# AnastasiaBelenkii/tendermint

Measured on AMD Instinct MI355X. Metric: ed25519 verifies/sec at 1/2/4/8 GPUs + p50 VerifyCommit latency, 150 vals, higher is better.
Workload: dtype int32

## Files before the change

__graft_entry__.py:

```python
import os
import subprocess
import sys

REPO = os.path.dirname(os.path.abspath(__file__))


def build() -> None:
    env = dict(os.environ, PYTORCH_ROCM_ARCH="gfx950")
    subprocess.run(["make", "-s", "-C", os.path.join(REPO, "tendermint_amd", "csrc")], check=True, env=env)
    subprocess.run(["bash", os.path.join(REPO, "tools", "build_checks.sh")], check=True, env=env)
    subprocess.run(["make", "-s", "-C", os.path.join(REPO, "oracle")], check=True)
    subprocess.run(["make", "-s", "-C", os.path.join(REPO, "tendermint_amd", "testing", "csrc")], check=True)
    subprocess.run(["make", "-s", "-C", os.path.join(REPO, "tests", "native")], check=True)
    subprocess.run(["make", "-s", "-C", os.path.join(REPO, "tests", "native", "secp")], check=True)
    subprocess.run(["make", "-s", "-C", os.path.join(REPO, "tests", "native", "secpcomb")], check=True)
    subprocess.run(["make", "-s", "-C", os.path.join(REPO, "tests", "native", "merkle")], check=True)
    subprocess.run(["make", "-s", "-C", os.path.join(REPO, "tests", "native", "pcache")], check=True)
    subprocess.run(["make", "-s", "-C", os.path.join(REPO, "tests", "native", "colorder")], check=True)
    subprocess.run(["make", "-s", "-C", os.path.join(REPO, "tests", "native", "blocks")], check=True)
    subprocess.run(["make", "-s", "-C", os.path.join(REPO, "tests", "native", "voteext")], check=True)
    subprocess.run(["make", "-s", "-C", os.path.join(REPO, "tests", "native", "proofops")], check=True)
    subprocess.run(["make", "-s", "-C", os.path.join(REPO, "tests", "native", "stage")], check=True)
    subprocess.run(["make", "-s", "-C", os.path.join(REPO, "tests", "native", "results")], check=True)
    sys.path.insert(0, REPO)
    import tendermint_amd
    from tendermint_amd import _native
    _native.lib()


def smoke() -> None:
    sys.path.insert(0, REPO)
    sys.path.insert(0, os.path.join(REPO, "oracle"))
    import numpy as np
    import torch
    from tendermint_amd import _native
    from tendermint_amd.testing.factory import make_c2_batch
    import oracle_c

    assert torch.cuda.is_available(), "smoke() needs a GPU"
    ctx = _native.Context(1)
    b = make_c2_batch(1000, seed=7)
    ok_g, vec_g = ctx.ed25519_verify_batch(b.pk, b.sig, b.msg, b.off)
    ok_o, vec_o = oracle_c.ed25519_verify_packed(b.pk, b.sig, b.msg, b.off, threads=4)
    assert ok_g == ok_o and np.array_equal(vec_g, vec_o), "GPU validity vector differs from the oracle"
    info = _native.build_info()
    print(f"smoke ok: {int(vec_g.sum())}/{b.n} valid, bit-exact vs oracle; {info['version']} "
          f"(src digest of this tree {'matches' if info['src_match'] else 'DIFFERS: ' + info['src_digest_tree']})")


if __name__ == "__main__":
    build()
    smoke()
```

include/tmverify.h:

```cpp
#ifndef TMVERIFY_H
#define TMVERIFY_H

#include <stddef.h>
#include <stdint.h>

#ifdef __cplusplus
extern "C" {
#endif

#define TMV_ALL_VALID 1
#define TMV_NOT_ALL 0
#define TMV_ERR_ARG (-1)
#define TMV_ERR_NO_DEVICE (-2)
#define TMV_ERR_NOMEM (-3)
#define TMV_ERR_LAUNCH (-4)
#define TMV_ERR_TIMEOUT (-5)
#define TMV_ERR_RANDOM (-6)

#define TMV_SR_ADDERR_PUBKEY (-1)
#define TMV_SR_ADDERR_SIG (-2)

#define TMV_KIND_ED25519 0
#define TMV_KIND_SR25519 1

// ... 9 lines not shown
int tmv_ed25519_verify_batch(tmv_ctx *ctx, const uint8_t *pk, const uint8_t *sig, const uint8_t *msg,
                             const uint32_t *msg_off, uint32_t n, uint8_t *valid_out);

int tmv_ed25519_verify(tmv_ctx *ctx, const uint8_t *pk, const uint8_t *msg, size_t msg_len,
                       const uint8_t *sig, size_t sig_len);

int tmv_secp256k1_verify_batch(tmv_ctx *ctx, const uint8_t *pk, const uint8_t *sig, const uint8_t *msg,
                               const uint32_t *msg_off, uint32_t n, uint8_t *valid_out);

int tmv_secp256k1_verify_batch_ex(tmv_ctx *ctx, uint32_t flags, const uint8_t *pk, const uint8_t *sig,
                                  const uint8_t *msg, const uint32_t *msg_off, uint32_t n, uint8_t *valid_out);
int tmv_secp256k1_key_cache_stats(tmv_ctx *ctx, uint64_t *hits, uint64_t *misses, uint32_t *used, uint32_t *capacity);

int tmv_secp256k1_verify(tmv_ctx *ctx, const uint8_t *pk, size_t pk_len, const uint8_t *msg, size_t msg_len,
                         const uint8_t *sig, size_t sig_len);

int tmv_sr25519_verify_batch(tmv_ctx *ctx, const uint8_t *pk, const uint8_t *sig, const uint8_t *msg,
                             const uint32_t *msg_off, uint32_t n, int8_t *status_out);

int tmv_verify_mixed_batch(tmv_ctx *ctx, const uint8_t *kind, const uint8_t *pk, const uint8_t *sig,
                           const uint8_t *msg, const uint32_t *msg_off, uint32_t n, int8_t *status_out);

#define TMV_FLAG_KEY_CACHE 1u
int tmv_verify_batch_ex(tmv_ctx *ctx, uint8_t key_kind, uint32_t flags, const uint8_t *pk, const uint8_t *sig,
                        const uint8_t *msg, const uint32_t *msg_off, uint32_t n, int8_t *status_out);
#define TMV_FLAG_BATCH_EQUATION 2u
#define TMV_FLAG_PER_ENTRY 4u
#define TMV_BATCHOPT_STATS 1u
#define TMV_BATCHOPT_SUBCHECK_ON 2u
#define TMV_BATCHOPT_SUBCHECK_OFF 4u
int tmv_set_batch_options(tmv_ctx *ctx, uint32_t group_log2, uint32_t window_bits, const uint8_t *seed32,
                          uint32_t opt_flags);
int tmv_batch_stats(tmv_ctx *ctx, uint64_t *groups, uint64_t *groups_failed);
int tmv_validator_set_hashes(tmv_ctx *ctx, const uint8_t *pk, const uint8_t *key_kind, const int64_t *power,
                             const uint32_t *set_off, uint32_t n_sets, uint8_t *hash_out);
int tmv_merkle_roots(tmv_ctx *ctx, const uint8_t *data, const uint32_t *leaf_off, uint32_t n_leaves,
                     const uint32_t *tree_off, uint32_t n_trees, uint8_t *hash_out);
int tmv_commit_hashes(tmv_ctx *ctx, const uint8_t *flag, const uint8_t *addr_len, const uint8_t *addr,
                      const int64_t *ts_seconds, const int32_t *ts_nanos, const uint8_t *sig_len, const uint8_t *sig,
                      const uint32_t *commit_off, uint32_t n_commits, uint8_t *hash_out);
#define TMV_RESULTS_FIRST_LEAF 1u
int tmv_tx_results_hashes(tmv_ctx *ctx, uint32_t flags, const uint32_t *code, const int64_t *gas_wanted,
                          const int64_t *gas_used, const uint8_t *data, const uint32_t *data_off,
                          const uint32_t *tree_off, uint32_t n_trees, const uint8_t *first, const uint32_t *first_off,
                          uint8_t *root_out);

#define TMV_MERKLE_PREHASH 1u
#define TMV_MERKLE_LEAF_HASH_GIVEN 2u
#define TMV_MERKLE_LONG_LEAVES 4u
#define TMV_MERKLE_SHORT_LEAVES 8u
#define TMV_MERKLE_LPW(l) ((uint32_t)(l) << 8)
int tmv_merkle_aunt_offsets(const uint32_t *tree_off, uint32_t n_trees, uint32_t *aunt_off_out);
int tmv_merkle_proofs(tmv_ctx *ctx, uint32_t flags, const uint8_t *data, const uint32_t *leaf_off, uint32_t n_leaves,
                      const uint32_t *tree_off, uint32_t n_trees, uint8_t *root_out, uint8_t *leaf_hash_out,
                      const uint32_t *aunt_off, uint8_t *aunts_out);
int tmv_merkle_verify_proofs(tmv_ctx *ctx, uint32_t flags, uint32_t n, const int64_t *total, const int64_t *index,
                             const uint8_t *leaf_hash, const uint8_t *aunts, const uint32_t *aunt_off,
                             const uint8_t *root, const uint8_t *data, const uint32_t *leaf_off, int8_t *status_out,
                             uint8_t *leaf_hash_calc, uint8_t *root_calc, uint8_t *root_nil);

int tmv_merkle_value_ops(tmv_ctx *ctx, uint32_t flags, uint32_t n_items, const uint8_t *value,
                         const uint32_t *value_off, const uint32_t *op_off, const uint8_t *key, const uint32_t *key_off,
                         const int64_t *total, const int64_t *index, const uint8_t *leaf_hash, const uint8_t *aunts,
                         const uint32_t *aunt_off, const uint8_t *root, uint8_t *value_digest, uint8_t *kv_hash_calc,
                         uint8_t *leaf_ok, uint8_t *root_calc, uint8_t *root_nil, int8_t *status_out,
                         int32_t *fail_op_out);

int tmv_subgroup_stats(tmv_ctx *ctx, uint64_t *subgroups, uint64_t *subgroups_failed);
int tmv_verify_mixed_batch_ex(tmv_ctx *ctx, uint32_t flags, const uint8_t *kind, const uint8_t *pk,
                              const uint8_t *sig, const uint8_t *msg, const uint32_t *msg_off, uint32_t n,
                              int8_t *status_out);

int tmv_kernel_timing(tmv_ctx *ctx, int enable);
int tmv_kernel_timing_read(tmv_ctx *ctx, const char *kernel, double *total_ms, uint64_t *launches);

int tmv_key_cache_stats(tmv_ctx *ctx, uint64_t *hits, uint64_t *misses, uint32_t *used, uint32_t *capacity);

int tmv_point_cache_stats(tmv_ctx *ctx, uint64_t *hits, uint64_t *misses, uint32_t *slots);

int tmv_bucket_entry_stats(tmv_ctx *ctx, uint64_t *entries);

int tmv_group_fail_stats(tmv_ctx *ctx, uint64_t *groups_failed, uint64_t *groups_located, uint64_t *fallback_entries);

typedef struct tmv_metrics {
  uint64_t calls;
  uint64_t signatures;
  uint64_t max_batch;
  uint64_t batch_eq_signatures;
  uint64_t host_signatures;
  double host_seconds;
  uint64_t h2d_bytes;
  uint64_t d2h_bytes;
  uint64_t groups;
  uint64_t groups_failed;
  uint64_t located_groups;
  uint64_t fallback_signatures;
  uint64_t key_cache_hits;
  uint64_t key_cache_misses;
} tmv_metrics;
int tmv_metrics_read(tmv_ctx *ctx, tmv_metrics *out);
int tmv_metrics_reset(tmv_ctx *ctx);

int tmv_ed25519_verify_batch_device(tmv_ctx *ctx, int device, const uint8_t *d_pk, const uint8_t *d_sig,
                                    const uint8_t *d_msg, const uint32_t *d_msg_off, uint32_t n,
                                    uint8_t *d_valid, void *stream);
int tmv_verify_mixed_batch_device(tmv_ctx *ctx, int device, const uint8_t *d_kind, const uint8_t *d_pk,
                                  const uint8_t *d_sig, const uint8_t *d_msg, const uint32_t *d_msg_off,
                                  uint32_t n, int8_t *d_status, void *stream);
#define TMV_KIND_MIXED 2
int tmv_verify_batch_device_ex(tmv_ctx *ctx, int device, uint8_t key_kind, uint32_t flags, const uint8_t *d_kind,
                               const uint8_t *d_pk, const uint8_t *d_sig, const uint8_t *d_msg,
                               const uint32_t *d_msg_off, uint32_t n, int8_t *d_status, void *stream);

#define TMV_MAX_BATCHES 256
typedef struct tmv_batch_ref {
  const uint8_t *pk;
  const uint8_t *sig;
  const uint8_t *msg;
  const uint32_t *msg_off;
  uint32_t n;
  uint32_t msg_bytes;
  int8_t *status;
} tmv_batch_ref;
int tmv_verify_batches_device(tmv_ctx *ctx, int device, uint8_t key_kind, uint32_t flags,
                              const tmv_batch_ref *batches, uint32_t n_batches, void *stream);

typedef struct tmv_vote_template {
  const uint8_t *head;
  uint32_t head_len;
  const uint8_t *block;
  uint32_t block_len;
  const uint8_t *chain;
  uint32_t chain_len;
} tmv_vote_template;

#define TMV_VOTE_WITH_BLOCK 0x80000000u

typedef struct tmv_vote {
  int64_t ts_seconds;
  int32_t ts_nanos;
  uint32_t tmpl;
} tmv_vote;

int tmv_verify_votes(tmv_ctx *ctx, uint8_t key_kind, uint32_t flags, const tmv_vote_template *tmpl,
                     uint32_t n_tmpl, const tmv_vote *votes, const uint8_t *pk, const uint8_t *sig, uint32_t n,
                     int8_t *status_out);

int64_t tmv_vote_sign_bytes_device(tmv_ctx *ctx, const tmv_vote_template *tmpl, uint32_t n_tmpl,
                                   const tmv_vote *votes, uint32_t n, uint8_t *msg_out, size_t msg_cap,
                                   uint32_t *msg_off_out);

typedef struct tmv_vote_ext_template { const uint8_t *tail; uint32_t tail_len; } tmv_vote_ext_template;

int tmv_verify_votes_and_extensions(tmv_ctx *ctx, uint8_t key_kind, uint32_t flags,
        const tmv_vote_template *tmpl, uint32_t n_tmpl, const tmv_vote *votes, uint32_t n_votes,
        const tmv_vote_ext_template *etmpl, uint32_t n_etmpl, const uint32_t *ext_tmpl,
        const uint8_t *ext_data, const uint32_t *ext_off, uint32_t n_exts,
        const uint8_t *pk, const uint8_t *sig, int8_t *status_out);
int64_t tmv_vote_extension_sign_bytes_device(tmv_ctx *ctx, const tmv_vote_ext_template *etmpl, uint32_t n_etmpl,
        const uint32_t *ext_tmpl, const uint8_t *ext_data, const uint32_t *ext_off, uint32_t n_exts,
        uint8_t *msg_out, size_t msg_cap, uint32_t *msg_off_out);

#ifdef __cplusplus
}
#endif
#endif
// ... 1 lines not shown
```

tendermint_amd/_native.py:

```python
from __future__ import annotations

import ctypes
import os
import subprocess
import threading

import numpy as np

_HERE = os.path.dirname(os.path.abspath(__file__))
LIB_PATH = os.environ.get("TMV_LIB_PATH") or os.path.join(_HERE, "_build", "libtmgpu.so")
HEADER_PATH = os.path.join(os.path.dirname(_HERE), "include", "tmverify.h")
HEADER_PATHS = [HEADER_PATH, os.path.join(os.path.dirname(_HERE), "include", "tmhost.h")]

TMV_ALL_VALID = 1
TMV_NOT_ALL = 0
TMV_ERR_ARG = -1
TMV_ERR_NO_DEVICE = -2
TMV_ERR_NOMEM = -3
TMV_ERR_LAUNCH = -4
TMV_SR_ADDERR_PUBKEY = -1
TMV_SR_ADDERR_SIG = -2
TMV_KIND_ED25519 = 0
TMV_KIND_SR25519 = 1
TMV_FLAG_KEY_CACHE = 1
TMV_FLAG_BATCH_EQUATION = 2
TMV_FLAG_PER_ENTRY = 4
TMV_BATCHOPT_STATS = 1
TMV_BATCHOPT_SUBCHECK_ON = 2
TMV_BATCHOPT_SUBCHECK_OFF = 4
TMV_MERKLE_PREHASH = 1
TMV_MERKLE_LEAF_HASH_GIVEN = 2
TMV_MERKLE_LONG_LEAVES = 4
TMV_MERKLE_SHORT_LEAVES = 8
TMV_RESULTS_FIRST_LEAF = 1
TMV_KIND_MIXED = 2
TMV_KIND_SECP256K1 = 3
TMV_VOTE_WITH_BLOCK = 0x80000000
VOTE_EXT_WAVE_MIN = 96

VOTE_DTYPE = np.dtype([("ts_seconds", "<i8"), ("ts_nanos", "<i4"), ("tmpl", "<u4")])

EXPORTS = [
    "tmv_open", "tmv_open_logical", "tmv_close", "tmv_num_devices", "tmv_last_error", "tmv_version",
    "tmv_ed25519_verify_batch", "tmv_ed25519_verify", "tmv_sr25519_verify_batch",
    "tmv_secp256k1_verify_batch", "tmv_secp256k1_verify", "tmv_secp256k1_verify_batch_ex",
    "tmv_secp256k1_key_cache_stats",
    "tmv_verify_mixed_batch", "tmv_ed25519_verify_batch_device", "tmv_verify_mixed_batch_device",
    "tmv_verify_batch_ex", "tmv_key_cache_stats", "tmv_point_cache_stats", "tmv_bucket_entry_stats", "tmv_group_fail_stats",
    "tmv_set_batch_options", "tmv_batch_stats",
    "tmv_subgroup_stats", "tmv_validator_set_hashes",
    "tmv_verify_mixed_batch_ex", "tmv_verify_batch_device_ex", "tmv_verify_batches_device",
    "tmv_verify_votes", "tmv_vote_sign_bytes_device", "tmv_verify_votes_and_extensions",
    "tmv_vote_extension_sign_bytes_device", "tmv_merkle_roots",
    "tmv_merkle_aunt_offsets", "tmv_merkle_proofs", "tmv_merkle_verify_proofs", "tmv_merkle_value_ops",
    "tmv_commit_hashes", "tmv_tx_results_hashes",
    "tmv_kernel_timing", "tmv_kernel_timing_read", "tmv_metrics_read", "tmv_metrics_reset",
    "tmv_batch_new", "tmv_batch_add", "tmv_batch_len", "tmv_batch_verify", "tmv_batch_free",
    "tmv_vote_sign_bytes", "tmv_vote_template_encode", "tmv_verify_commit", "tmv_verify_commits",
    "tmv_header_hashes", "tmv_light_verify_many", "tmv_light_verify", "tmv_verify_vote_batch",
    "tmv_part_set_headers", "tmv_part_set_proofs", "tmv_parts_verify", "tmv_proofs_verify",
    "tmv_proof_ops_verify", "tmv_tx_proofs_validate",
    "tmv_commit_hash_many", "tmv_blocks_validate_basic",
    "tmv_results_hash_many", "tmv_consensus_params_hash", "tmv_block_results_verify", "tmv_consensus_params_verify",
    "tmv_vote_extension_sign_bytes", "tmv_vote_extension_template_encode", "tmv_verify_extended_votes",
]


class BatchRef(ctypes.Structure):
    _fields_ = [("pk", ctypes.c_void_p), ("sig", ctypes.c_void_p), ("msg", ctypes.c_void_p),
                ("msg_off", ctypes.c_void_p), ("n", ctypes.c_uint32), ("msg_bytes", ctypes.c_uint32),
                ("status", ctypes.c_void_p)]


class Metrics(ctypes.Structure):
    _fields_ = [("calls", ctypes.c_uint64), ("signatures", ctypes.c_uint64), ("max_batch", ctypes.c_uint64),
                ("batch_eq_signatures", ctypes.c_uint64), ("host_signatures", ctypes.c_uint64),
                ("host_seconds", ctypes.c_double), ("h2d_bytes", ctypes.c_uint64), ("d2h_bytes", ctypes.c_uint64),
                ("groups", ctypes.c_uint64), ("groups_failed", ctypes.c_uint64),
                ("located_groups", ctypes.c_uint64), ("fallback_signatures", ctypes.c_uint64),
                ("key_cache_hits", ctypes.c_uint64), ("key_cache_misses", ctypes.c_uint64)]


class VoteTemplate(ctypes.Structure):
    _fields_ = [("head", ctypes.c_void_p), ("head_len", ctypes.c_uint32), ("block", ctypes.c_void_p),
                ("block_len", ctypes.c_uint32), ("chain", ctypes.c_void_p), ("chain_len", ctypes.c_uint32)]


def vote_templates(segments):
    keep = []
    arr = (VoteTemplate * max(1, len(segments)))()
    for t, segs in enumerate(segments):
        ptrs = []
        for b in segs:
            buf = ctypes.create_string_buffer(bytes(b), max(1, len(b)))
            keep.append(buf)
            ptrs.append((ctypes.cast(buf, ctypes.c_void_p), len(b)))
        arr[t] = VoteTemplate(ptrs[0][0], ptrs[0][1], ptrs[1][0], ptrs[1][1], ptrs[2][0], ptrs[2][1])
    return arr, keep


class VoteExtTemplate(ctypes.Structure):
    _fields_ = [("tail", ctypes.c_void_p), ("tail_len", ctypes.c_uint32)]


def vote_ext_templates(tails):
    keep = []
    arr = (VoteExtTemplate * max(1, len(tails)))()
    for t, b in enumerate(tails):
        buf = ctypes.create_string_buffer(bytes(b), max(1, len(b)))
        keep.append(buf)
        arr[t] = VoteExtTemplate(ctypes.cast(buf, ctypes.c_void_p), len(b))
    return arr, keep


def _ext_args(ext_tmpl, ext_data, ext_off):
    ext_tmpl = np.ascontiguousarray(ext_tmpl, np.uint32)
    ext_off = np.ascontiguousarray(ext_off, np.uint32)
    ext_data = np.ascontiguousarray(ext_data, np.uint8)
    if len(ext_off) != len(ext_tmpl) + 1:
        raise ValueError("ext_off must hold one more entry than ext_tmpl")
    return ext_tmpl, (ext_data if len(ext_data) else np.zeros(1, np.uint8)), ext_off


class NativeError(RuntimeError):
    pass


def build() -> str:
    subprocess.run(["make", "-s", "-C", os.path.join(_HERE, "csrc")], check=True)
    return LIB_PATH


_lib = None
_lib_lock = threading.Lock()


def lib() -> ctypes.CDLL:
    global _lib
    with _lib_lock:
        if _lib is not None:
            return _lib
        if not os.path.exists(LIB_PATH):
            raise NativeError(f"{LIB_PATH} missing: run tendermint_amd._native.build() "
                              "(there is no CPU fallback)")
        L = ctypes.CDLL(LIB_PATH)
        u8p = ctypes.POINTER(ctypes.c_uint8)
        i8p = ctypes.POINTER(ctypes.c_int8)
        u32p = ctypes.POINTER(ctypes.c_uint32)
        vp = ctypes.c_void_p
        L.tmv_open.restype = vp
        L.tmv_open.argtypes = [ctypes.c_uint32]
        L.tmv_open_logical.restype = vp
        L.tmv_open_logical.argtypes = [ctypes.c_uint32, ctypes.c_int]
        L.tmv_close.argtypes = [vp]
        L.tmv_num_devices.argtypes = [vp]
        L.tmv_last_error.restype = ctypes.c_char_p
        L.tmv_version.restype = ctypes.c_char_p
        L.tmv_ed25519_verify_batch.argtypes = [vp, u8p, u8p, u8p, u32p, ctypes.c_uint32, u8p]
        L.tmv_ed25519_verify.argtypes = [vp, u8p, u8p, ctypes.c_size_t, u8p, ctypes.c_size_t]
        L.tmv_secp256k1_verify_batch.argtypes = [vp, u8p, u8p, u8p, u32p, ctypes.c_uint32, u8p]
        L.tmv_secp256k1_verify.argtypes = [vp, u8p, ctypes.c_size_t, u8p, ctypes.c_size_t, u8p, ctypes.c_size_t]
        L.tmv_secp256k1_verify_batch_ex.argtypes = [vp, ctypes.c_uint32, u8p, u8p, u8p, u32p, ctypes.c_uint32, u8p]
        L.tmv_secp256k1_key_cache_stats.argtypes = [vp, ctypes.POINTER(ctypes.c_uint64),
                                                    ctypes.POINTER(ctypes.c_uint64), ctypes.POINTER(ctypes.c_uint32),
                                                    ctypes.POINTER(ctypes.c_uint32)]
        L.tmv_sr25519_verify_batch.argtypes = [vp, u8p, u8p, u8p, u32p, ctypes.c_uint32, i8p]
        L.tmv_verify_mixed_batch.argtypes = [vp, u8p, u8p, u8p, u8p, u32p, ctypes.c_uint32, i8p]
        L.tmv_verify_batch_ex.argtypes = [vp, ctypes.c_uint8, ctypes.c_uint32, u8p, u8p, u8p, u32p, ctypes.c_uint32,
                                          i8p]
        L.tmv_key_cache_stats.argtypes = [vp, ctypes.POINTER(ctypes.c_uint64), ctypes.POINTER(ctypes.c_uint64),
                                          ctypes.POINTER(ctypes.c_uint32), ctypes.POINTER(ctypes.c_uint32)]
        L.tmv_point_cache_stats.argtypes = [vp, ctypes.POINTER(ctypes.c_uint64), ctypes.POINTER(ctypes.c_uint64),
                                            ctypes.POINTER(ctypes.c_uint32)]
        L.tmv_bucket_entry_stats.argtypes = [vp, ctypes.POINTER(ctypes.c_uint64)]
        L.tmv_group_fail_stats.argtypes = [vp] + [ctypes.POINTER(ctypes.c_uint64)] * 3
        L.tmv_set_batch_options.argtypes = [vp, ctypes.c_uint32, ctypes.c_uint32, u8p, ctypes.c_uint32]
        L.tmv_batch_stats.argtypes = [vp, ctypes.POINTER(ctypes.c_uint64), ctypes.POINTER(ctypes.c_uint64)]
        L.tmv_kernel_timing.argtypes = [vp, ctypes.c_int]
        L.tmv_kernel_timing_read.argtypes = [vp, ctypes.c_char_p, ctypes.POINTER(ctypes.c_double),
                                             ctypes.POINTER(ctypes.c_uint64)]
        L.tmv_subgroup_stats.argtypes = [vp, ctypes.POINTER(ctypes.c_uint64), ctypes.POINTER(ctypes.c_uint64)]
        L.tmv_validator_set_hashes.argtypes = [vp, u8p, u8p, ctypes.POINTER(ctypes.c_int64), u32p,
                                               ctypes.c_uint32, u8p]
        L.tmv_verify_mixed_batch_ex.argtypes = [vp, ctypes.c_uint32, u8p, u8p, u8p, u8p, u32p, ctypes.c_uint32, i8p]
        L.tmv_merkle_roots.argtypes = [vp, u8p, u32p, ctypes.c_uint32, u32p, ctypes.c_uint32, u8p]
        L.tmv_merkle_aunt_offsets.argtypes = [u32p, ctypes.c_uint32, u32p]
        L.tmv_commit_hashes.argtypes = [vp, u8p, u8p, u8p, ctypes.POINTER(ctypes.c_int64),
                                        ctypes.POINTER(ctypes.c_int32), u8p, u8p, u32p, ctypes.c_uint32, u8p]
        L.tmv_merkle_proofs.argtypes = [vp, ctypes.c_uint32, u8p, u32p, ctypes.c_uint32, u32p, ctypes.c_uint32, u8p,
                                        u8p, u32p, u8p]
        i64p = ctypes.POINTER(ctypes.c_int64)
        L.tmv_tx_results_hashes.argtypes = [vp, ctypes.c_uint32, u32p, i64p, i64p, u8p, u32p, u32p, ctypes.c_uint32,
                                            u8p, u32p, u8p]
        L.tmv_merkle_verify_proofs.argtypes = [vp, ctypes.c_uint32, ctypes.c_uint32, i64p, i64p, u8p, u8p, u32p, u8p,
                                               u8p, u32p, i8p, u8p, u8p, u8p]
        L.tmv_merkle_value_ops.argtypes = [vp, ctypes.c_uint32, ctypes.c_uint32, u8p, u32p, u32p, u8p, u32p, i64p, i64p,
                                           u8p, u8p, u32p, u8p, u8p, u8p, u8p, u8p, u8p, i8p,
                                           ctypes.POINTER(ctypes.c_int32)]
        L.tmv_verify_batch_device_ex.argtypes = [vp, ctypes.c_int, ctypes.c_uint8, ctypes.c_uint32, vp, vp, vp, vp,
                                                 vp, ctypes.c_uint32, vp, vp]
        L.tmv_verify_batches_device.argtypes = [vp, ctypes.c_int, ctypes.c_uint8, ctypes.c_uint32,
                                                ctypes.POINTER(BatchRef), ctypes.c_uint32, vp]
        L.tmv_verify_votes.argtypes = [vp, ctypes.c_uint8, ctypes.c_uint32, ctypes.POINTER(VoteTemplate),
                                       ctypes.c_uint32, vp, u8p, u8p, ctypes.c_uint32, i8p]
        L.tmv_vote_sign_bytes_device.restype = ctypes.c_int64
        L.tmv_vote_sign_bytes_device.argtypes = [vp, ctypes.POINTER(VoteTemplate), ctypes.c_uint32, vp,
                                                 ctypes.c_uint32, u8p, ctypes.c_size_t, u32p]
        L.tmv_verify_votes_and_extensions.argtypes = [vp, ctypes.c_uint8, ctypes.c_uint32,
                                                      ctypes.POINTER(VoteTemplate), ctypes.c_uint32, vp, ctypes.c_uint32,
                                                      ctypes.POINTER(VoteExtTemplate), ctypes.c_uint32, u32p, u8p, u32p,
                                                      ctypes.c_uint32, u8p, u8p, i8p]
        L.tmv_vote_extension_sign_bytes_device.restype = ctypes.c_int64
        L.tmv_vote_extension_sign_bytes_device.argtypes = [vp, ctypes.POINTER(VoteExtTemplate), ctypes.c_uint32, u32p,
                                                           u8p, u32p, ctypes.c_uint32, u8p, ctypes.c_size_t, u32p]
        L.tmv_ed25519_verify_batch_device.argtypes = [vp, ctypes.c_int, vp, vp, vp, vp, ctypes.c_uint32, vp, vp]
        L.tmv_verify_mixed_batch_device.argtypes = [vp, ctypes.c_int, vp, vp, vp, vp, vp, ctypes.c_uint32, vp, vp]
        L.tmv_metrics_read.argtypes = [vp, ctypes.POINTER(Metrics)]
        L.tmv_metrics_reset.argtypes = [vp]
        _lib = L
        return L


def merkle_lpw(leaves_per_wave: int) -> int:
    return leaves_per_wave << 8


def merkle_aunt_offsets(tree_off: np.ndarray) -> np.ndarray:
    tree_off = np.ascontiguousarray(tree_off, np.uint32)
    out = np.zeros(int(tree_off[-1]) + 1, np.uint32)
    rc = lib().tmv_merkle_aunt_offsets(_p(tree_off, ctypes.c_uint32), len(tree_off) - 1, _p(out, ctypes.c_uint32))
    if rc < 0:
        raise NativeError(f"tmv_merkle_aunt_offsets failed ({rc}): {last_error()}")
    return out


def last_error() -> str:
    return lib().tmv_last_error().decode(errors="replace")


def version() -> str:
    return lib().tmv_version().decode(errors="replace")


def build_info() -> dict:
    import importlib.util
    v = version()
    fields = dict(kv.split("=", 1) for kv in v.split() if "=" in kv)
    spec = importlib.util.spec_from_file_location("tmv_src_digest", os.path.join(_HERE, "csrc", "src_digest.py"))
    mod = importlib.util.module_from_spec(spec)
    spec.loader.exec_module(mod)
    tree = mod.digest()
    return {"version": v, "src_digest_compiled": fields.get("src"), "src_digest_tree": tree,
            "src_match": fields.get("src") == tree, "git_head_compiled": fields.get("git"),
            "library": LIB_PATH}


def _p(a: np.ndarray, t=ctypes.c_uint8):
    return a.ctypes.data_as(ctypes.POINTER(t))
# ... 332 lines not shown
    def merkle_value_ops(self, value, value_off, op_off, key, key_off, total, index, leaf_hash, aunts, aunt_off, root,
                         flags: int = 0, skip=()):
        value_off = np.ascontiguousarray(value_off, np.uint32)
        op_off = np.ascontiguousarray(op_off, np.uint32)
        key_off = np.ascontiguousarray(key_off, np.uint32)
        aunt_off = np.ascontiguousarray(aunt_off, np.uint32)
        n_items, n_ops = len(op_off) - 1, len(key_off) - 1

        def data(a, width=1):
            if a is None:
                return None
            a = np.ascontiguousarray(a, np.uint8)
            return a if a.size else np.zeros(width, np.uint8)

        value, key, aunts = data(value), data(key), data(aunts, 32)
        leaf_hash, root = data(leaf_hash, 32), data(root, 32)
        total = np.ascontiguousarray(total, np.int64) if n_ops else np.zeros(1, np.int64)
        index = np.ascontiguousarray(index, np.int64) if n_ops else np.zeros(1, np.int64)
        out = {"value_digest": np.zeros((max(n_items, 1), 32), np.uint8),
               "kv_hash_calc": np.zeros((max(n_ops, 1), 32), np.uint8),
               "leaf_ok": np.zeros(max(n_ops, 1), np.uint8),
               "root_calc": np.zeros((max(n_ops, 1), 32), np.uint8),
               "root_nil": np.zeros(max(n_ops, 1), np.uint8),
               "status": np.zeros(max(n_items, 1), np.int8),
               "fail_op": np.zeros(max(n_items, 1), np.int32)}
        types = {"status": ctypes.c_int8, "fail_op": ctypes.c_int32}
        ptr = {k: (None if k in skip else _p(v, types.get(k, ctypes.c_uint8))) for k, v in out.items()}

        def opt(a):
            return None if a is None else _p(a)

        rc = self._check(self._lib.tmv_merkle_value_ops(
            self._h, flags, n_items, opt(value), _p(value_off, ctypes.c_uint32), _p(op_off, ctypes.c_uint32), opt(key),
            _p(key_off, ctypes.c_uint32), _p(total, ctypes.c_int64), _p(index, ctypes.c_int64), opt(leaf_hash),
            opt(aunts), _p(aunt_off, ctypes.c_uint32), opt(root), ptr["value_digest"], ptr["kv_hash_calc"],
            ptr["leaf_ok"], ptr["root_calc"], ptr["root_nil"], ptr["status"], ptr["fail_op"]),
            "tmv_merkle_value_ops")
        size = {"value_digest": n_items, "status": n_items, "fail_op": n_items}
        return rc == 0, {k: (None if k in skip else v[:size.get(k, n_ops)]) for k, v in out.items()}

    def batch_stats(self):
        g, f = ctypes.c_uint64(), ctypes.c_uint64()
        self._check(self._lib.tmv_batch_stats(self._h, ctypes.byref(g), ctypes.byref(f)), "tmv_batch_stats")
        sg, sf = ctypes.c_uint64(), ctypes.c_uint64()
        self._check(self._lib.tmv_subgroup_stats(self._h, ctypes.byref(sg), ctypes.byref(sf)), "tmv_subgroup_stats")
        return {"groups": g.value, "failed": f.value, "subgroups": sg.value, "sub_failed": sf.value}

    def verify_batch_device_ex(self, device: int, key_kind: int, flags: int, d_kind: int, d_pk: int, d_sig: int,
                               d_msg: int, d_off: int, n: int, d_status: int, stream: int = 0) -> None:
        self._check(self._lib.tmv_verify_batch_device_ex(self._h, device, key_kind, flags, d_kind or None, d_pk,
                                                         d_sig, d_msg, d_off, n, d_status, stream or None),
                    "tmv_verify_batch_device_ex")

    def verify_batches_device(self, device: int, key_kind: int, flags: int, refs, stream: int = 0) -> None:
        arr = (BatchRef * len(refs))(*refs)
        self._check(self._lib.tmv_verify_batches_device(self._h, device, key_kind, flags, arr, len(refs),
                                                        stream or None), "tmv_verify_batches_device")

    def key_cache_stats(self):
        h, m = ctypes.c_uint64(), ctypes.c_uint64()
        u, c = ctypes.c_uint32(), ctypes.c_uint32()
        self._check(self._lib.tmv_key_cache_stats(self._h, ctypes.byref(h), ctypes.byref(m), ctypes.byref(u),
                                                  ctypes.byref(c)), "tmv_key_cache_stats")
        return {"hits": h.value, "misses": m.value, "used": u.value, "capacity": c.value}

    def point_cache_stats(self):
        h, m = ctypes.c_uint64(), ctypes.c_uint64()
        c = ctypes.c_uint32()
        self._check(self._lib.tmv_point_cache_stats(self._h, ctypes.byref(h), ctypes.byref(m), ctypes.byref(c)),
                    "tmv_point_cache_stats")
        return {"hits": h.value, "misses": m.value, "slots": c.value}

    def bucket_entry_stats(self) -> int:
        v = ctypes.c_uint64()
        self._check(self._lib.tmv_bucket_entry_stats(self._h, ctypes.byref(v)), "tmv_bucket_entry_stats")
        return v.value

    def group_fail_stats(self) -> dict:
        f, l, e = ctypes.c_uint64(), ctypes.c_uint64(), ctypes.c_uint64()
        self._check(self._lib.tmv_group_fail_stats(self._h, ctypes.byref(f), ctypes.byref(l), ctypes.byref(e)),
                    "tmv_group_fail_stats")
        return {"failed": f.value, "located": l.value, "fallback_entries": e.value}

    def metrics(self) -> dict:
        m = Metrics()
        self._check(self._lib.tmv_metrics_read(self._h, ctypes.byref(m)), "tmv_metrics_read")
        d = {k: getattr(m, k) for k, _ in Metrics._fields_}
        d["verifies_per_s_host"] = d["host_signatures"] / d["host_seconds"] if d["host_seconds"] else 0.0
        return d

    def metrics_reset(self) -> None:
        self._check(self._lib.tmv_metrics_reset(self._h), "tmv_metrics_reset")

    def ed25519_verify_batch_device(self, device: int, d_pk: int, d_sig: int, d_msg: int, d_off: int, n: int,
                                    d_valid: int, stream: int = 0) -> None:
        self._check(self._lib.tmv_ed25519_verify_batch_device(self._h, device, d_pk, d_sig, d_msg, d_off, n,
                                                              d_valid, stream or None),
                    "tmv_ed25519_verify_batch_device")

    def verify_mixed_batch_device(self, device: int, d_kind: int, d_pk: int, d_sig: int, d_msg: int, d_off: int,
                                  n: int, d_status: int, stream: int = 0) -> None:
        self._check(self._lib.tmv_verify_mixed_batch_device(self._h, device, d_kind, d_pk, d_sig, d_msg, d_off, n,
                                                            d_status, stream or None),
                    "tmv_verify_mixed_batch_device")


_default_ctx = None
_ctx_lock = threading.Lock()


def default_context() -> Context:
    global _default_ctx
    with _ctx_lock:
        if _default_ctx is None:
            _default_ctx = Context(0)
        return _default_ctx
```

tendermint_amd/csrc/msm.h:

```cpp
#pragma once
#include <stdint.h>
#include "curve25519.h"

namespace tmv {

constexpr uint32_t kMsmWideRows = 65536;
constexpr int kMsmChunkMax = 32;
constexpr uint32_t kMsmEmpty = 0xffffffffu;
constexpr uint32_t kMsmCompactGroups = 2048;
constexpr int kMsmSortBlock = 256;
constexpr uint32_t kSubGroupLog2 = 3;
constexpr uint32_t kSubGroup = 1u << kSubGroupLog2;

struct alignas(16) niels_pt {
  fe ypx, ymx, xy2d;
  int32_t pad[2];
};

#ifndef TMV_NIELS_PAIR
#define TMV_NIELS_PAIR 0
#endif
constexpr uint32_t kNielsPer = TMV_NIELS_PAIR ? 2 : 1;

TMV_HD niels_pt niels_negate(const niels_pt &p) {
  niels_pt r;
  r.ypx = p.ymx;
  r.ymx = p.ypx;
  fe_neg(r.xy2d, p.xy2d);
  r.pad[0] = r.pad[1] = 0;
  return r;
}

TMV_HD void niels_store(niels_pt *pts, uint64_t i, const niels_pt &p) {
  if (kNielsPer == 2) {
    pts[2 * i] = p;
    pts[2 * i + 1] = niels_negate(p);
  } else {
    pts[i] = p;
  }
}

struct MsmParams {
  uint32_t m_log2;
  uint32_t c;
  uint32_t W;
  uint32_t WR;
  uint32_t H;
  uint32_t cap;
  uint32_t groups;
  uint32_t P;
  uint32_t L;
  uint32_t merged;
  uint32_t sub;

  TMV_HD uint32_t m() const { return 1u << m_log2; }
  TMV_HD uint32_t WL() const { return (129 + m_log2 + c - 1) / c; }
  TMV_HD uint32_t buckets_per_group() const { return W * H; }
  TMV_HD uint32_t bucket(uint32_t w, uint32_t i) const { return w * H + i; }
  TMV_HD uint32_t chunks_per_group() const { return cap / L; }
  TMV_HD uint32_t wpart_slots() const { return P; }

  static MsmParams make(uint32_t n, uint32_t m_log2, uint32_t c, bool merged = false) {
    MsmParams p;
    p.m_log2 = m_log2;
    p.c = c;
    p.merged = merged ? 1 : 0;
    p.sub = 0;
    p.WR = (129 + c - 1) / c;
    p.W = merged ? p.WR : (254 + c - 1) / c;
    p.H = 1u << (c - 1);
    const uint32_t m = 1u << m_log2;
    const uint32_t rw = p.WR > p.WL() ? p.WR : p.WL();
    const uint32_t slots = merged ? m * p.WR : m * rw + (m + 1) * p.W;
    p.cap = (slots + kMsmChunkMax - 1) / kMsmChunkMax * kMsmChunkMax;
    const uint32_t mean = (merged ? m : 2 * m) / p.H;
    p.L = mean <= 16 ? 16 : 32;
    p.groups = (n + m - 1) >> m_log2;
    uint32_t best = ~0u;
    for (uint32_t P = 1; P <= p.H; P *= 2) {
      uint32_t lg = 0;
      while ((p.H / P) >> (lg + 1)) lg++;
      const uint32_t chain = 2 * (p.H / P) + 3 * P + lg;
      if (chain < best) { best = chain; p.P = P; }
    }
    if ((uint64_t)p.groups * p.W >= kMsmWideRows) p.P = 1;
    return p;
  }
};

struct MsmWork {
  niels_pt *pts;
  uint32_t *ent_pt;
  uint32_t *ent_bk;
  uint32_t *bk_start;
  uint32_t *bk_cnt;
  ge_p3 *bk_sum;
  ge_p3 *part_first;
  ge_p3 *part_last;
  uint32_t *join_b;
  uint32_t *join_count;
  ge_p3 *wpart;
  ge_p3 *wsum;
  uint32_t *grp_chunks;
  uint32_t *chunk_end;
  uint32_t compact;
  uint8_t *group_ok;
  uint8_t *sort_ovf;
  uint32_t n_pts;
  uint32_t *fail_count;
  uint32_t *fail_list;
  uint8_t *sub_ok;
  fe *tabR;
  fe *fail_T;
  uint32_t *loc_count;
  uint32_t *fb_count;
  uint32_t *loc_found;
  uint32_t *fb_list;
  const uint8_t *merge_pk;
  unsigned long long *ent_total;
  uint32_t *wscal;
  uint32_t *bscal;
  fe *item_pt;

  static size_t max_items(uint32_t n, const MsmParams &p) { return (size_t)n + 2ull * p.groups; }

  static size_t bytes(uint32_t n, const MsmParams &p) {
    const size_t G = p.groups, bk = (size_t)G * p.buckets_per_group(), ent = (size_t)G * p.cap;
    const size_t chunks = ent / p.L;
    size_t b = (2ull * n + 1) * kNielsPer * sizeof(niels_pt) + 8 * ent + 8 * bk + bk * sizeof(ge_p3) +
               2 * chunks * sizeof(ge_p3) + 4 * chunks + G * p.W * (2ull * p.wpart_slots() + 1) * sizeof(ge_p3) + G + 2 * G +
               18 * 16 + 4 * G + 8 * G + 32;
    if (p.merged) b += 32ull * n + 32 * G + max_items(n, p) * 4 * sizeof(fe);
    else b += 16 + 4 * G + (G << p.m_log2) / kSubGroup + 16 + (size_t)n * 32 * sizeof(fe) + 3 * 16 +
              G * 8 * sizeof(fe) + 16 + 4ull * n + 2 * 16 + 4 * G + 2 * 16 + G * 4 * sizeof(fe) + 16;
    return b;
  }
  static MsmWork carve(void *base, uint32_t n, const MsmParams &p) {
    auto up = [](size_t x) { return (x + 15) & ~size_t(15); };
    uint8_t *b = static_cast<uint8_t *>(base);
    const size_t G = p.groups, bk = (size_t)G * p.buckets_per_group(), ent = (size_t)G * p.cap;
    const size_t chunks = ent / p.L;
    MsmWork w;
    size_t o = 0;
    w.pts = reinterpret_cast<niels_pt *>(b + o); o = up(o + (2ull * n + 1) * kNielsPer * sizeof(niels_pt));
    w.ent_pt = reinterpret_cast<uint32_t *>(b + o); o = up(o + 4 * ent);
    w.ent_bk = reinterpret_cast<uint32_t *>(b + o); o = up(o + 4 * ent);
    w.bk_start = reinterpret_cast<uint32_t *>(b + o); o = up(o + 4 * bk);
    w.bk_cnt = reinterpret_cast<uint32_t *>(b + o); o = up(o + 4 * bk);
    w.bk_sum = reinterpret_cast<ge_p3 *>(b + o); o = up(o + bk * sizeof(ge_p3));
    w.part_first = reinterpret_cast<ge_p3 *>(b + o); o = up(o + chunks * sizeof(ge_p3));
    w.part_last = reinterpret_cast<ge_p3 *>(b + o); o = up(o + chunks * sizeof(ge_p3));
    w.join_b = reinterpret_cast<uint32_t *>(b + o); o = up(o + 4 * chunks);
    w.join_count = reinterpret_cast<uint32_t *>(b + o); o = up(o + 4 * G);
    w.wpart = reinterpret_cast<ge_p3 *>(b + o); o = up(o + G * p.W * 2ull * p.wpart_slots() * sizeof(ge_p3));
    w.wsum = reinterpret_cast<ge_p3 *>(b + o); o = up(o + G * p.W * sizeof(ge_p3));
    w.grp_chunks = reinterpret_cast<uint32_t *>(b + o); o = up(o + 4 * G);
    w.chunk_end = reinterpret_cast<uint32_t *>(b + o); o = up(o + 4 * G);
    w.group_ok = b + o; o = up(o + G);
    w.sort_ovf = b + o; o = up(o + 2 * G);
    w.n_pts = 2 * n;
    w.merge_pk = nullptr;
    w.compact = 0;
    w.ent_total = nullptr;
    w.wscal = w.bscal = nullptr;
    w.item_pt = nullptr;
    w.fail_count = w.fail_list = nullptr;
    w.sub_ok = nullptr;
    w.tabR = nullptr;
    w.fail_T = nullptr;
    w.loc_count = w.fb_count = w.fb_list = w.loc_found = nullptr;
    if (!p.merged) {
      w.fail_count = reinterpret_cast<uint32_t *>(b + o); o = up(o + 16);
      w.fail_list = reinterpret_cast<uint32_t *>(b + o); o = up(o + 4 * G);
      w.sub_ok = b + o; o = up(o + (G << p.m_log2) / kSubGroup);
      w.tabR = reinterpret_cast<fe *>(b + o); o = up(o + (size_t)n * 32 * sizeof(fe));
      w.fail_T = reinterpret_cast<fe *>(b + o); o = up(o + G * 8 * sizeof(fe));
      w.loc_count = reinterpret_cast<uint32_t *>(b + o);
      w.fb_count = w.loc_count + 1;
      w.loc_found = w.loc_count + 2;
      o = up(o + 16);
      w.fb_list = reinterpret_cast<uint32_t *>(b + o); o = up(o + 4ull * n);
    }
    if (p.merged) {
      w.wscal = reinterpret_cast<uint32_t *>(b + o); o = up(o + 32ull * n);
      w.bscal = reinterpret_cast<uint32_t *>(b + o); o = up(o + 32 * G);
      w.item_pt = reinterpret_cast<fe *>(b + o);
    }
    return w;
  }
};

struct MsmSeed {
  uint32_t key[8];
  uint32_t nonce[3];
};

TMV_HD uint32_t rotl32(uint32_t x, int n) { return (x << n) | (x >> (32 - n)); }

#define TMV_QR(a, b, c, d)              \
  a += b; d ^= a; d = rotl32(d, 16);    \
  c += d; b ^= c; b = rotl32(b, 12);    \
  a += b; d ^= a; d = rotl32(d, 8);     \
  c += d; b ^= c; b = rotl32(b, 7);

TMV_HD void chacha20_block(uint32_t out[16], const uint32_t key[8], uint32_t counter, const uint32_t nonce[3]) {
  uint32_t x[16];
  x[0] = 0x61707865u; x[1] = 0x3320646eu; x[2] = 0x79622d32u; x[3] = 0x6b206574u;
#pragma unroll
  for (int i = 0; i < 8; i++) x[4 + i] = key[i];
  x[12] = counter;
  x[13] = nonce[0]; x[14] = nonce[1]; x[15] = nonce[2];
  uint32_t s[16];
#pragma unroll
  for (int i = 0; i < 16; i++) s[i] = x[i];
#pragma unroll 1
  for (int r = 0; r < 10; r++) {
    TMV_QR(s[0], s[4], s[8], s[12]);
    TMV_QR(s[1], s[5], s[9], s[13]);
    TMV_QR(s[2], s[6], s[10], s[14]);
    TMV_QR(s[3], s[7], s[11], s[15]);
    TMV_QR(s[0], s[5], s[10], s[15]);
    TMV_QR(s[1], s[6], s[11], s[12]);
    TMV_QR(s[2], s[7], s[8], s[13]);
    TMV_QR(s[3], s[4], s[9], s[14]);
  }
#pragma unroll
  for (int i = 0; i < 16; i++) out[i] = s[i] + x[i];
}
#undef TMV_QR

TMV_HD void niels_to_p3(ge_p3 &r, const fe &ypx, const fe &ymx) {
  fe e, h;
  fe_sub(e, ypx, ymx);
  fe_add(h, ypx, ymx);
  fe_mul(r.T, e, h);
  fe_add(e, e, e);
  fe_add(h, h, h);
  fe_carry(r.X, e);
  fe_carry(r.Y, h);
  fe_zero(r.Z);
  r.Z.v[0] = 4;
}

TMV_HD void sc_mul_mod(uint32_t r[8], const uint32_t *a, int na, const uint32_t b[8]) {
  uint32_t x[16];
#pragma unroll
  for (int i = 0; i < 16; i++) x[i] = 0;
#pragma unroll
  for (int i = 0; i < na; i++) {
    uint64_t carry = 0;
#pragma unroll
    for (int j = 0; j < 8; j++) {
      const uint64_t t = (uint64_t)a[i] * b[j] + x[i + j] + carry;
      x[i + j] = (uint32_t)t;
      carry = t >> 32;
    }
    x[i + 8] = (uint32_t)carry;
  }
  sc_reduce512(r, x);
}

TMV_HD int sc_window_digit(const uint32_t *s, int nw, uint32_t w, uint32_t c, bool top, int &carry) {
  const uint32_t bit = w * c;
  const uint32_t wi = bit >> 5, sh = bit & 31;
  uint64_t x = wi < (uint32_t)nw ? s[wi] : 0;
  if (wi + 1 < (uint32_t)nw) x |= (uint64_t)s[wi + 1] << 32;
  int d = (int)((x >> sh) & ((1u << c) - 1)) + carry;
  if (!top && d >= (1 << (c - 1))) {
    d -= 1 << c;
    carry = 1;
// ... 8 lines not shown
```

tendermint_amd/csrc/msm_kernels.hip:

```cpp
#include <hip/hip_runtime.h>
#include <cstdlib>
#include <cstring>
#include "ed25519_core.h"
#include "kernel_util.h"
#include "comb.h"
#include "quad.h"
#include "ktimer.h"
#include "verify_kernels.h"
#include "halfscalar.h"
#include "knobs.h"

#include <algorithm>
#include <atomic>
#include <mutex>
#include <vector>

namespace tmv {

namespace ktimer {
namespace {
struct Pair {
  int k;
  hipEvent_t a, b;
};
// ... 44 lines not shown
  }
  int rc = 0;
  for (Pair *p : v) {
    float t = 0.f;
    hipError_t e = hipEventSynchronize(p->b);
    if (e == hipSuccess) e = hipEventElapsedTime(&t, p->a, p->b);
    if (e == hipSuccess) {
      *ms += t;
      *launches += 1;
    } else if (!rc) {
      rc = (int)e;
    }
    std::lock_guard<std::mutex> lk(g_mu);
    g_free.push_back(p->a);
    g_free.push_back(p->b);
    delete p;
  }
  return rc;
}

}

namespace {

template <int V>
struct StaticIndex {
  static constexpr int value = V;
};

template <int NW>
struct DigitReader {
  uint32_t wd[NW];
  uint64_t buf;
  uint32_t avail;
  int carry;
  __device__ __forceinline__ void init(const uint32_t *s) {
#pragma unroll
    for (int k = 0; k < NW; k++) wd[k] = s[k];
    buf = 0;
    avail = 0;
    carry = 0;
  }
  __device__ __forceinline__ int next(uint32_t c, bool top) {
    if (avail < c) {
      buf |= (uint64_t)wd[0] << avail;
#pragma unroll
      for (int k = 0; k + 1 < NW; k++) wd[k] = wd[k + 1];
      wd[NW - 1] = 0;
      avail += 32;
    }
    int d = (int)(buf & ((1u << c) - 1)) + carry;
    buf >>= c;
    avail -= c;
    if (!top && d >= (1 << (c - 1))) {
      d -= 1 << c;
      carry = 1;
    } else {
      carry = 0;
    }
    return d;
  }
};

template <int NW, typename F>
__device__ __forceinline__ void for_each_digit(const uint32_t *s, uint32_t windows, const MsmParams &p, F f) {
  DigitReader<NW> rd;
  rd.init(s);
  for (uint32_t w = 0; w < windows; w++) {
    const int d = rd.next(p.c, w + 1 == windows);
    if (d != 0) f(p.bucket(w, (uint32_t)((d < 0 ? -d : d) - 1)), d < 0);
  }
}

__device__ __forceinline__ void p3_add(ge_p3 &a, const ge_p3 &b) {
  ge_cached c;
  ge_p3_to_cached(c, b);
  ge_p1p1 r;
  ge_add(r, a, c);
  ge_p1p1_to_p3(a, r);
}

TMV_HD uint32_t merge_runs(const MsmParams &p) { return p.m() / 2 < 256u ? p.m() / 2 : 256u; }

__device__ __forceinline__ void p3_dbl(ge_p3 &a) {
  ge_p1p1 r;
  ge_p3_dbl(r, a);
  ge_p1p1_to_p3(a, r);
}

}

template <bool SR, bool KM, int BS = kMsmSortBlock, bool LOC = false>
__global__ void __launch_bounds__(BS)
k_msm_sort(const uint8_t *__restrict__ sig, const uint32_t *__restrict__ idx, const uint32_t *count_ptr, uint32_t n,
           Ed25519Work w, MsmWork mw, MsmParams p, MsmSeed seed, const fe *__restrict__ btab_q, int aligned,
           const uint32_t *__restrict__ key_slot, const uint8_t *__restrict__ key_ok, uint8_t *__restrict__ out,
           uint32_t e_base) {
  extern __shared__ uint32_t smem[];
  const uint32_t cnt = entry_count(count_ptr, n);
  const uint32_t tid = threadIdx.x;
  uint32_t g = blockIdx.x;
  if (g == 0 && tid == 0) *mw.join_count = 0;
  if (LOC) {
    const uint32_t nf = *mw.fail_count;
    if (g == 0 && tid == 0) {
      *mw.loc_count = nf << p.m_log2;
      *mw.fb_count = 0;
      *mw.loc_found = 0;
    }
    if (g >= nf) return;
  }
  const uint32_t slot = g;
  if (LOC) g = mw.fail_list[slot];
  const uint32_t e0 = g << p.m_log2;
  if (!KM && !LOC && g == 0 && tid == 0) {
    niels_pt bp;
    bp.ymx = btab_q[0];
    bp.ypx = btab_q[1];
    bp.xy2d = btab_q[2];
    bp.pad[0] = bp.pad[1] = 0;
    niels_store(mw.pts, mw.n_pts, bp);
    if (mw.fail_count) *mw.fail_count = 0;
  }
  if (e0 >= cnt) return;
  const uint32_t mlive = min(p.m(), cnt - e0);
  const uint32_t WH = p.W * p.H;
  uint32_t *hist = smem;
  uint32_t *red = smem + WH;
  uint32_t *scan = red + BS * 9;

  constexpr int R = 4;
  constexpr int ZW = LOC ? 5 : 4;
  const uint32_t WRz = LOC ? p.WL() : p.WR;
  uint32_t z[R][ZW], wv[R][8];
  bool live[R];
  uint32_t acc[9];
#pragma unroll
  for (int t = 0; t < 9; t++) acc[t] = 0;
  auto weigh = [&](auto rc) {
    constexpr int r = decltype(rc)::value;
    live[r] = false;
#pragma unroll
    for (int t = 0; t < ZW; t++) z[r][t] = 0;
#pragma unroll
    for (int t = 0; t < 8; t++) wv[r][t] = 0;
    const uint32_t j = tid + r * BS;
    if (j >= mlive) return;
    const uint32_t e = e0 + j;
    const uint32_t i = idx ? idx[e] : e;
    uint32_t s_raw[8], s[8];
    if (aligned) load_words_aligned(s_raw, sig + 64ull * i + 32);
    else load_words_unaligned(s_raw, sig + 64ull * i + 32);
    bool s_ok;
    if (SR) {
      s_ok = sr25519_decode_s(s, s_raw);
    } else {
#pragma unroll
      for (int t = 0; t < 8; t++) s[t] = s_raw[t];
      s_ok = sc_is_canonical(s);
    }
    const bool a_ok = KM ? key_ok[key_slot[i]] != 0 : w.flags[4 * e] != 0;
    if (!KM && !LOC && out) {
      const bool r_ok = w.flags[4 * e + 1] != 0;
      const int st = SR ? (!a_ok ? -1 : (!s_ok ? -2 : (r_ok ? 1 : 0))) : ((a_ok && r_ok && s_ok) ? 1 : 0);
      out[i] = (uint8_t)(int8_t)st;
    }
    if (!(s_ok && a_ok && w.flags[4 * e + 1])) {
      if (KM) {
        uint4 *wd = reinterpret_cast<uint4 *>(mw.wscal + 8ull * e);
        wd[0] = wd[1] = make_uint4(0, 0, 0, 0);
      }
      return;
    }
    live[r] = true;
    uint32_t blk[16];
    chacha20_block(blk, seed.key, e_base + e, seed.nonce);
#pragma unroll
    for (int t = 0; t < 4; t++) z[r][t] = blk[t];
    uint32_t k[8];
    const uint4 *kp = reinterpret_cast<const uint4 *>(w.k + 8ull * e);
    const uint4 k0 = kp[0], k1 = kp[1];
    k[0] = k0.x; k[1] = k0.y; k[2] = k0.z; k[3] = k0.w;
    k[4] = k1.x; k[5] = k1.y; k[6] = k1.z; k[7] = k1.w;
    sc_mul_mod(wv[r], z[r], 4, k);
    if constexpr (LOC) {
      const uint32_t jj = j + 1;
      uint64_t cy = 0;
#pragma unroll
      for (int t = 0; t < 4; t++) {
        cy += (uint64_t)z[r][t] * jj;
        z[r][t] = (uint32_t)cy;
        cy >>= 32;
      }
      z[r][4] = (uint32_t)cy;
      uint32_t t8[8];
#pragma unroll
      for (int t = 0; t < 8; t++) t8[t] = wv[r][t];
      sc_mul_mod(wv[r], &jj, 1, t8);
    }
    if (KM) {
      uint4 *wd = reinterpret_cast<uint4 *>(mw.wscal + 8ull * e);
      wd[0] = make_uint4(wv[r][0], wv[r][1], wv[r][2], wv[r][3]);
      wd[1] = make_uint4(wv[r][4], wv[r][5], wv[r][6], wv[r][7]);
    }
// ... 66 lines not shown
#pragma unroll
      for (int r = 0; r < R; r++) {
        myslot[r] = 0;
        if (!live[r]) continue;
        uint32_t kw[8];
        key_words(kw, tid + r * BS);
        uint32_t tag = 0x811c9dc5u;
#pragma unroll
        for (int t = 0; t < 8; t++) tag = (tag ^ kw[t]) * 0x01000193u + (tag >> 15);
        tag |= 1u;
        uint32_t h = (tag * 0x9e3779b1u) >> tshift;
        for (;;) {
          const uint32_t old = atomicCAS(&ttag[h], 0u, tag);
          if (old == 0 || old == tag) break;
          h = (h + 1) & tmask;
        }
        atomicMin(&tlead[h], tid + r * BS);
        myslot[r] = h;
      }
      __syncthreads();
      bool follower[R], leader[R];
#pragma unroll
      for (int r = 0; r < R; r++) {
        follower[r] = leader[r] = false;
        if (!live[r]) continue;
        const uint32_t lead = tlead[myslot[r]];
        leader[r] = lead == tid + r * BS;
        if (leader[r]) continue;
        uint32_t kw[8], lw[8];
        key_words(kw, tid + r * BS);
        key_words(lw, lead);
        uint32_t diff = 0;
#pragma unroll
        for (int t = 0; t < 8; t++) diff |= kw[t] ^ lw[t];
        if (diff) continue;
        follower[r] = true;
        trun[myslot[r]] = kWant;
      }
      __syncthreads();
#pragma unroll
      for (int r = 0; r < R; r++) {
        if (!leader[r] || trun[myslot[r]] != kWant) continue;
        const uint32_t sl = atomicAdd(nruns, 1u);
        trun[myslot[r]] = sl < RUNS ? sl : kNone;
      }
      __syncthreads();
#pragma unroll
      for (int r = 0; r < R; r++) {
        if (!follower[r]) continue;
        const uint32_t sl = trun[myslot[r]];
        if (sl >= RUNS) continue;
#pragma unroll
        for (int t = 0; t < 8; t++) {
          atomicAdd(&racc[sl * 16 + 2 * t], wv[r][t] & 0xffffu);
          atomicAdd(&racc[sl * 16 + 2 * t + 1], wv[r][t] >> 16);
          wv[r][t] = 0;
        }
      }
      __syncthreads();
#pragma unroll
      for (int r = 0; r < R; r++) {
        if (!leader[r]) continue;
        const uint32_t sl = trun[myslot[r]];
        if (sl >= RUNS) continue;
        uint32_t x[16];
        uint64_t c = 0;
#pragma unroll
        for (int t = 0; t < 8; t++) {
          c += (uint64_t)racc[sl * 16 + 2 * t] + (wv[r][t] & 0xffffu);
          const uint32_t lo16 = (uint32_t)c & 0xffffu;
          c >>= 16;
          c += (uint64_t)racc[sl * 16 + 2 * t + 1] + (wv[r][t] >> 16);
          x[t] = lo16 | (((uint32_t)c & 0xffffu) << 16);
          c >>= 16;
        }
        x[8] = (uint32_t)c;
#pragma unroll
        for (int t = 9; t < 16; t++) x[t] = 0;
        sc_reduce512(wv[r], x);
      }
    }
  }

#pragma unroll
  for (int r = 0; r < R; r++) {
    if (!live[r]) continue;
    for_each_digit<ZW>(z[r], WRz, p, [&](uint32_t bk, bool) { atomicAdd(&hist[bk], 1u); });
    if (!KM) for_each_digit<8>(wv[r], p.W, p, [&](uint32_t bk, bool) { atomicAdd(&hist[bk], 1u); });
  }
  if (!KM && tid == 0) for_each_digit<8>(bsc, p.W, p, [&](uint32_t bk, bool) { atomicAdd(&hist[bk], 1u); });
  __syncthreads();

  const uint32_t seg = (WH + BS - 1) / BS;
  const uint32_t lo = min(WH, tid * seg), hi = min(WH, lo + seg);
  uint32_t local = 0;
  for (uint32_t t = lo; t < hi; t++) local += hist[t];
  scan[tid] = local;
  __syncthreads();
  if (tid == 0) {
    uint32_t run = 0;
    for (int t = 0; t < BS; t++) {
      const uint32_t v = scan[t];
      scan[t] = run;
      run += v;
    }
    scan[BS] = run;
  }
  __syncthreads();
  const uint32_t gbase = slot * p.cap;
  const uint32_t bbase = slot * WH;
  const bool ovf = scan[BS] > p.cap;
  if (tid == 0) mw.sort_ovf[(LOC ? p.groups : 0) + slot] = ovf ? 1 : 0;
  if (tid == 0 && !ovf && mw.ent_total) atomicAdd(mw.ent_total, (unsigned long long)scan[BS]);
  if (tid == 0) mw.grp_chunks[slot] = ovf ? 0u : (scan[BS] + p.L - 1) / p.L;
  if (ovf) {
    for (uint32_t t = tid; t < WH; t += BS) {
      mw.bk_start[bbase + t] = gbase;
      mw.bk_cnt[bbase + t] = 0;
    }
    for (uint32_t t = tid; t < p.cap; t += BS) mw.ent_bk[gbase + t] = kMsmEmpty;
    return;
  }
  {
    uint32_t off = scan[tid];
    for (uint32_t t = lo; t < hi; t++) {
      const uint32_t c = hist[t];
      mw.bk_start[bbase + t] = gbase + off;
      mw.bk_cnt[bbase + t] = c;
      hist[t] = off;
      off += c;
    }
  }
  __syncthreads();

  uint32_t *ent_pt = mw.ent_pt + gbase;
  uint32_t *ent_bk = mw.ent_bk + gbase;
  const uint32_t wcap = 2 * p.m() + 1;
  uint32_t *st_pt = scan + BS + 1, *st_bk = st_pt + wcap;
  DigitReader<ZW> rz[R];
  DigitReader<8> rw[R], rb;
#pragma unroll
  for (int r = 0; r < R; r++) {
    rz[r].init(z[r]);
    rw[r].init(wv[r]);
  }
  rb.init(bsc);
  const uint32_t total = scan[BS];
  for (uint32_t w = 0; w < p.W; w++) {
    const uint32_t wbeg = hist[p.bucket(w, 0)];
    const uint32_t wend = w + 1 < p.W ? hist[p.bucket(w + 1, 0)] : total;
    __syncthreads();
#pragma unroll
    for (int r = 0; r < R; r++) {
      if (!live[r]) continue;
      const uint32_t e = e0 + tid + r * BS;
      if (w < WRz) {
        const int d = rz[r].next(p.c, w + 1 == WRz);
        if (d != 0) {
          const uint32_t bk = p.bucket(w, (uint32_t)((d < 0 ? -d : d) - 1));
          const uint32_t pos = atomicAdd(&hist[bk], 1u) - wbeg;
          st_pt[pos] = ((KM ? e : 2 * e) << 1) | (d < 0 ? 1u : 0u);
          st_bk[pos] = bbase + bk;
        }
      }
      if (!KM) {
        const int d = rw[r].next(p.c, w + 1 == p.W);
        if (d != 0) {
          const uint32_t bk = p.bucket(w, (uint32_t)((d < 0 ? -d : d) - 1));
          const uint32_t pos = atomicAdd(&hist[bk], 1u) - wbeg;
          st_pt[pos] = ((2 * e + 1) << 1) | (d < 0 ? 1u : 0u);
          st_bk[pos] = bbase + bk;
        }
      }
    }
    if (!KM && tid == 0) {
      const int d = rb.next(p.c, w + 1 == p.W);
      if (d != 0) {
        const uint32_t bk = p.bucket(w, (uint32_t)((d < 0 ? -d : d) - 1));
        const uint32_t pos = atomicAdd(&hist[bk], 1u) - wbeg;
        st_pt[pos] = (mw.n_pts << 1) | (d < 0 ? 1u : 0u);
        st_bk[pos] = bbase + bk;
      }
    }
    __syncthreads();
    for (uint32_t i = tid; i < wend - wbeg; i += BS) {
      ent_pt[wbeg + i] = st_pt[i];
      ent_bk[wbeg + i] = st_bk[i];
    }
  }
  const uint32_t pad_end = mw.compact ? min(p.cap, (total + p.L - 1) / p.L * p.L) : p.cap;
  for (uint32_t t = total + tid; t < pad_end; t += BS) ent_bk[t] = kMsmEmpty;
}

#ifdef TMV_CHECKS
__device__ uint32_t g_joins_named, g_joins_done, g_buckets_unwritten;
#endif

template <int L>
__global__ void __launch_bounds__(256)
k_msm_accum(const uint32_t *count_ptr, uint32_t n, MsmWork mw, MsmParams p) {
  __shared__ ge_p3 first_run[256];
  const uint32_t cpg = p.chunks_per_group();
  const uint32_t live_groups = (entry_count(count_ptr, n) + p.m() - 1) >> p.m_log2;
  if (live_groups == 0) return;
  const uint32_t total = mw.chunk_end ? mw.chunk_end[live_groups - 1] : live_groups * cpg;
  const uint32_t live_blocks = (total + blockDim.x - 1) / blockDim.x;
  const uint32_t per_xcd = (live_blocks + 7) / 8;
  if ((blockIdx.x >> 3) >= per_xcd) return;
  const uint32_t lb = (blockIdx.x & 7) * per_xcd + (blockIdx.x >> 3);
  uint32_t t = lb * blockDim.x + threadIdx.x;
  if (mw.chunk_end) {
    if (lb * blockDim.x >= total) return;
    uint32_t lo = 0, hi = live_groups - 1;
    while (lo < hi) {
      const uint32_t mid = (lo + hi) >> 1;
      if (mw.chunk_end[mid] > lb * blockDim.x) hi = mid;
      else lo = mid + 1;
    }
    if (t >= total) return;
    uint32_t gc = lo;
    while (gc + 1 < live_groups && mw.chunk_end[gc] <= t) gc++;
    const uint32_t off = t - (gc ? mw.chunk_end[gc - 1] : 0u);
    if (off >= cpg) return;
    t = gc * cpg + off;
  }
  const uint32_t g = t / cpg;
  if (g >= live_groups) return;
  const uint32_t base = t * L;
  const uint32_t lane = threadIdx.x & 63;
  uint32_t bk[L], pt[L];
  {
    const uint4 *b4 = reinterpret_cast<const uint4 *>(mw.ent_bk + base);
    const uint4 *p4 = reinterpret_cast<const uint4 *>(mw.ent_pt + base);
#pragma unroll
    for (int q = 0; q < L / 4; q++) {
      const uint4 x = b4[q], y = p4[q];
      bk[4 * q] = x.x; bk[4 * q + 1] = x.y; bk[4 * q + 2] = x.z; bk[4 * q + 3] = x.w;
      pt[4 * q] = y.x; pt[4 * q + 1] = y.y; pt[4 * q + 2] = y.z; pt[4 * q + 3] = y.w;
    }
  }
  if (bk[0] == kMsmEmpty) return;
  uint32_t join = kMsmEmpty;
  auto flush = [&](uint32_t b, uint32_t rs, uint32_t re, const ge_p3 &acc) {
    const uint32_t bs = mw.bk_start[b], be = bs + mw.bk_cnt[b];
    if (rs == bs && re == be) {
      mw.bk_sum[b] = acc;
    } else if (re == base + L && re < be) {
      mw.part_last[t] = acc;
    } else if (lane != 0 && bs >= base - L) {
      first_run[threadIdx.x] = acc;
    } else {
      mw.part_first[t] = acc;
      join = b;
    }
  };
  ge_p3 acc;
  const uint32_t pt0 = pt[0];
  if (kNielsPer == 2) {
    const niels_pt P = mw.pts[pt0];
    niels_to_p3(acc, P.ypx, P.ymx);
  } else {
    const niels_pt P = mw.pts[pt0 >> 1];
    const bool neg = pt0 & 1;
    niels_to_p3(acc, neg ? P.ymx : P.ypx, neg ? P.ypx : P.ymx);
  }
  uint32_t cur = bk[0], rs = base;
  uint32_t j = 1;
  bool more = true;
  uint32_t bn = bk[1], pn = pt[1];
#pragma unroll
  for (int q = 1; q < L; q++) {
    const uint32_t bq = bn, pq = pn;
    if (q + 1 < L) {
      bn = bk[q + 1];
// ... 35 lines not shown
  asm volatile("s_waitcnt lgkmcnt(0)" ::: "memory");
  __builtin_amdgcn_wave_barrier();
  __builtin_amdgcn_fence(__ATOMIC_ACQUIRE, "wavefront");
  if (join_next) {
    p3_add(acc, first_run[threadIdx.x + 1]);
    mw.bk_sum[cur] = acc;
  }
  const uint64_t jm = __ballot(join != kMsmEmpty);
  if (jm) {
    const int leader = __ffsll((unsigned long long)jm) - 1;
    uint32_t jb = 0;
    if ((int)lane == leader) jb = atomicAdd(mw.join_count, (uint32_t)__popcll(jm));
    jb = __shfl(jb, leader);
    if (join != kMsmEmpty) mw.join_b[jb + __popcll(jm & ((1ull << lane) - 1))] = join;
#ifdef TMV_CHECKS
    if ((int)lane == leader) atomicAdd(&g_joins_named, (uint32_t)__popcll(jm));
#endif
  }
}

constexpr int kScanBlock = 1024;
__global__ void __launch_bounds__(kScanBlock)
k_msm_chunk_scan(const uint32_t *count_ptr, uint32_t n, MsmWork mw, MsmParams p) {
  __shared__ uint32_t part[kScanBlock];
  const uint32_t live_groups = (entry_count(count_ptr, n) + p.m() - 1) >> p.m_log2;
  const uint32_t cpg = p.chunks_per_group();
  const uint32_t seg = (live_groups + kScanBlock - 1) / kScanBlock;
  const uint32_t lo = min(live_groups, threadIdx.x * seg), hi = min(live_groups, lo + seg);
  uint32_t sum = 0;
  for (uint32_t g = lo; g < hi; g++) sum += min(mw.grp_chunks[g], cpg);
  part[threadIdx.x] = sum;
  __syncthreads();
  for (uint32_t d = 1; d < kScanBlock; d <<= 1) {
    const uint32_t v = threadIdx.x >= d ? part[threadIdx.x - d] : 0;
    __syncthreads();
    part[threadIdx.x] += v;
    __syncthreads();
  }
  uint32_t run = part[threadIdx.x] - sum;
  for (uint32_t g = lo; g < hi; g++) {
    run += min(mw.grp_chunks[g], cpg);
    mw.chunk_end[g] = run;
  }
}

__global__ void __launch_bounds__(256)
k_msm_join_list(MsmWork mw, MsmParams p) {
  const uint32_t cnt = *mw.join_count;
  for (uint32_t i = blockIdx.x * blockDim.x + threadIdx.x; i < cnt; i += gridDim.x * blockDim.x) {
    const uint32_t b = mw.join_b[i];
    const uint32_t bs = mw.bk_start[b], t0 = bs / p.L, t1 = (bs + mw.bk_cnt[b] - 1) / p.L;
    ge_p3 acc = mw.part_last[t0];
    for (uint32_t t = t0 + 1; t < t1; t++) {
      const ge_p3 q = mw.part_last[t];
      p3_add(acc, q);
    }
    const ge_p3 q = mw.part_first[t1];
    p3_add(acc, q);
    mw.bk_sum[b] = acc;
#ifdef TMV_CHECKS
    atomicAdd(&g_joins_done, 1u);
#endif
  }
}


__device__ __forceinline__ void store_window_sum(ge_p3 *dst, const ge_p3 &S, bool top) {
  if (top) {
    *dst = S;
    return;
  }
  ge_p3 q;
  fe t;
  fe_sub(t, S.Y, S.X);
  fe_carry(q.X, t);
  fe_add(t, S.Y, S.X);
  fe_carry(q.Y, t);
  fe_mul(q.Z, S.T, consts::d2());
  q.T = S.Z;
  *dst = q;
}

__global__ void __launch_bounds__(256)
k_msm_wpart(const uint32_t *count_ptr, uint32_t n, MsmWork mw, MsmParams p) {
  const uint32_t t = blockIdx.x * blockDim.x + threadIdx.x;
  const uint32_t per_group = p.W * p.P;
  const uint32_t g = t / per_group;
  if (g >= p.groups || (g << p.m_log2) >= entry_count(count_ptr, n)) return;
  const uint32_t r = t - g * per_group, wdx = r / p.P, part = r % p.P;
  const uint32_t s = p.H / p.P;
  ge_p3 U, T;
  bool u_set = false, t_set = false;
  const uint32_t gb = g * p.W * p.H, i0 = part * s;
  if (p.P == 1) {
    ge_cached Uc;
    uint32_t cnt = mw.bk_cnt[gb + p.bucket(wdx, s - 1)];
    for (int i = (int)s - 1; i >= 0; i--) {
      const uint32_t c_i = cnt;
      if (i > 0) cnt = mw.bk_cnt[gb + p.bucket(wdx, (uint32_t)i - 1)];
      ge_p1p1 rr;
      bool first = false;
      if (c_i) {
        const ge_p3 B = mw.bk_sum[gb + p.bucket(wdx, (uint32_t)i)];
        if (u_set) {
          ge_add(rr, B, Uc);
          ge_p1p1_to_cached(Uc, rr);
        } else {
          ge_p3_to_cached(Uc, B);
          T = B;
          u_set = t_set = first = true;
        }
      }
      if (u_set && !first) {
        ge_add(rr, T, Uc);
        ge_p1p1_to_p3(T, rr);
      }
    }
  } else {
    uint32_t cnt = mw.bk_cnt[gb + p.bucket(wdx, i0 + s - 1)];
    for (int i = (int)s - 1; i >= 0; i--) {
      const uint32_t c_i = cnt;
      if (i > 0) cnt = mw.bk_cnt[gb + p.bucket(wdx, i0 + (uint32_t)i - 1)];
      if (c_i) {
        const ge_p3 B = mw.bk_sum[gb + p.bucket(wdx, i0 + (uint32_t)i)];
        if (u_set) p3_add(U, B);
        else { U = B; u_set = true; }
      }
      if (u_set) {
        if (t_set) p3_add(T, U);
        else { T = U; t_set = true; }
      }
    }
  }
  if (!u_set) ge_p3_identity(U);
  if (!t_set) ge_p3_identity(T);
  if (p.P > 1) {
    mw.wpart[2ull * t] = T;
    mw.wpart[2ull * t + 1] = U;
  } else {
    store_window_sum(&mw.wpart[2ull * t], T, wdx == p.W - 1);
  }
}

__global__ void __launch_bounds__(256)
k_msm_wsum(const uint32_t *count_ptr, uint32_t n, MsmWork mw, MsmParams p) {
  const uint32_t t = blockIdx.x * blockDim.x + threadIdx.x;
  const uint32_t g = t / p.W;
  if (g >= p.groups || (g << p.m_log2) >= entry_count(count_ptr, n)) return;
  const ge_p3 *wp = mw.wpart + 2ull * t * p.P;
  ge_p3 acc;
  if (p.P > 1) {
    ge_p3 r = wp[2 * (p.P - 1) + 1];
    acc = r;
    for (uint32_t q = p.P - 2; q >= 1; q--) {
      p3_add(r, wp[2 * q + 1]);
      p3_add(acc, r);
    }
    for (uint32_t d = p.H / p.P; d > 1; d >>= 1) p3_dbl(acc);
    for (uint32_t q = 0; q < p.P; q++) p3_add(acc, wp[2 * q]);
  } else {
    acc = wp[0];
  }
  store_window_sum(&mw.wsum[t], acc, t - g * p.W == p.W - 1);
}

template <bool SR, bool KM, bool LOC>
__device__ __forceinline__ void horner_block(uint32_t bx, const uint32_t *count_ptr, uint32_t n, MsmWork mw,
                                             const MsmParams &p, const uint32_t *__restrict__ group_run0,
                                             uint32_t n_runs) {
  const uint32_t live_groups = (entry_count(count_ptr, n) + p.m() - 1) >> p.m_log2;
  if (bx * 16 >= live_groups) return;
  const uint32_t raw = bx * 16 + (threadIdx.x >> 2);
  const bool live = raw < live_groups;
  const uint32_t g = live ? raw : live_groups - 1;
  const int c = (int)(threadIdx.x & 3);
  const uint32_t st = p.P == 1 ? 2 : 1;
  const ge_p3 *S = p.P == 1 ? mw.wpart + 2ull * g * p.W : mw.wsum + (size_t)g * p.W;
  fe acc = reinterpret_cast<const fe *>(&S[st * (p.W - 1)])[c];
  fe r, q, qc;
  for (int wI = (int)p.W - 2; wI >= 0; wI--) {
    qc = reinterpret_cast<const fe *>(&S[st * wI])[c];
    for (uint32_t d = 0; d < p.c; d++) {
      quad::dbl(r, acc);
      quad::p1p1_to_p3(acc, r);
    }
    quad::add(r, acc, qc);
    quad::p1p1_to_p3(acc, r);
  }
  if (KM) {
    const uint32_t r0 = group_run0[g], r1 = group_run0[g + 1];
    for (uint32_t it = r0; it <= r1; it++) {
      q = mw.item_pt[4ull * (it < r1 ? it : n_runs + g) + c];
      quad::to_cached(qc, q);
      quad::add(r, acc, qc);
      quad::p1p1_to_p3(acc, r);
    }
  }
  if (LOC) {
    if (live) mw.fail_T[8ull * g + 4 + c] = acc;
    return;
  }
  bool ok;
  if (SR) {
    fe id;
    quad::p3_identity(id);
    ok = quad::ristretto_equal(acc, id);
  } else {
    ok = quad::is_identity_times8(acc);
  }
  ok = ok && !mw.sort_ovf[g];
  int f = -1;
  if (live && c == 0) {
    mw.group_ok[g] = ok ? 1 : 0;
    if (!ok && mw.fail_list) {
      f = (int)atomicAdd(mw.fail_count, 1u);
      mw.fail_list[f] = g;
    }
  }
  f = __builtin_amdgcn_mov_dpp(f, quad::qp(0, 0, 0, 0), 0xF, 0xF, false);
  if (f >= 0 && mw.fail_T) mw.fail_T[8ull * f + c] = acc;
}

template <bool SR, bool KM, bool LOC = false>
__global__ void __launch_bounds__(64)
k_msm_horner(const uint32_t *count_ptr, uint32_t n, MsmWork mw, MsmParams p, const uint32_t *__restrict__ group_run0,
             uint32_t n_runs) {
  horner_block<SR, KM, LOC>(blockIdx.x, count_ptr, n, mw, p, group_run0, n_runs);
}

template <bool SR>
__global__ void __launch_bounds__(64)
k_msm_horner_helped(const uint32_t *count_ptr, uint32_t n, MsmWork mw, MsmParams p, Ed25519Work w,
                    uint32_t hblocks) {
  if (blockIdx.x < hblocks) {
    __builtin_amdgcn_s_setprio(3);
    horner_block<SR, false, false>(blockIdx.x, count_ptr, n, mw, p, nullptr, 0u);
    return;
  }
  const uint32_t e = (blockIdx.x - hblocks) * 64 + threadIdx.x;
  if (e >= entry_count(count_ptr, n)) return;
  const uint4 *kp = reinterpret_cast<const uint4 *>(w.k + 8ull * e);
  const uint4 k0 = kp[0], k1 = kp[1];
  const uint32_t k[8] = {k0.x, k0.y, k0.z, k0.w, k1.x, k1.y, k1.z, k1.w};
  uint32_t u[4], v[4];
  bool neg = false;
  const bool fast = half::reduce(u, neg, v, k);
  uint4 *hd = reinterpret_cast<uint4 *>(w.hs_buf + 12ull * e);
  hd[0] = make_uint4(u[0], u[1], u[2], u[3]);
  hd[1] = make_uint4(v[0], v[1], v[2], v[3]);
  hd[2] = make_uint4((fast ? 1u : 0u) | (neg ? 2u : 0u), 0u, 0u, 0u);
}

template <bool SR>
__global__ void __launch_bounds__(64)
k_loc_search(const uint32_t *count_ptr, uint32_t n, MsmWork mw, MsmParams p) {
  __shared__ int s_cnt, s_j;
  __shared__ uint32_t s_base;
  const uint32_t f = blockIdx.x;
  if (f >= *mw.fail_count) return;
  const int c = (int)(threadIdx.x & 3), q = (int)(threadIdx.x >> 2);
  if (threadIdx.x == 0) {
    s_cnt = 0;
    s_j = -1;
  }
  fe M = mw.fail_T[8ull * f + c], Mp = mw.fail_T[8ull * f + 4 + c], r;
  if (!SR) {
    for (int i = 0; i < 3; i++) {
      quad::dbl(r, M);
      quad::p1p1_to_p3(M, r);
      quad::dbl(r, Mp);
      quad::p1p1_to_p3(Mp, r);
    }
  }
  fe Mc, Dc, P = M, D = M;
  quad::to_cached(Mc, M);
  const int k = q + 1;
  for (int b = 30 - __builtin_clz((unsigned)k); b >= 0; b--) {
    quad::dbl(r, P);
    quad::p1p1_to_p3(P, r);
    if ((k >> b) & 1) {
      quad::add(r, P, Mc);
      quad::p1p1_to_p3(P, r);
    }
  }
  for (int i = 0; i < 4; i++) {
    quad::dbl(r, D);
    quad::p1p1_to_p3(D, r);
  }
  quad::to_cached(Dc, D);
  __syncthreads();
  const uint32_t m = p.m();
  for (uint32_t j = (uint32_t)q; j < m; j += 16) {
    const bool eq = SR ? quad::ristretto_equal(P, Mp) : quad::p3_equal(P, Mp);
    if (eq && c == 0) {
      atomicAdd(&s_cnt, 1);
      s_j = (int)j;
    }
    quad::add(r, P, Dc);
    quad::p1p1_to_p3(P, r);
  }
  __syncthreads();
  const uint32_t e0 = mw.fail_list[f] << p.m_log2;
  const uint32_t mlive = min(m, entry_count(count_ptr, n) - e0);
  const bool ovf = mw.sort_ovf[p.groups + f];
  if (s_cnt == 1 && (uint32_t)s_j < mlive && !ovf) {
    if (threadIdx.x == 0) {
      mw.fb_list[atomicAdd(mw.fb_count, 1u)] = e0 + (uint32_t)s_j;
      atomicAdd(mw.loc_found, 1u);
    }
    return;
// ... 106 lines not shown
      const niels_pt &np = mw.pts[(2ull * e + ra) * kNielsPer];
      fe E, H, P;
      fe_sub(E, np.ypx, np.ymx);
      fe_add(H, np.ypx, np.ymx);
      fe_mul(P, E, H);
      if (c == 0) { fe_add(E, E, E); fe_carry(P, E); }
      else if (c == 1) { fe_add(H, H, H); fe_carry(P, H); }
      else if (c == 2) { fe_zero(P); P.v[0] = 4; }
      fe *tab = (ra ? w.tabA : mw.tabR) + 32ull * e;
      fe r, Pm, Q, Q0;
      quad::to_cached(Q0, P);
      tab[c] = Q0;
      quad::dbl(r, P);
      quad::p1p1_to_p3(Pm, r);
      quad::to_cached(Q, Pm);
      tab[4 + c] = Q;
      for (int m = 2; m < 8; m++) {
        quad::add(r, Pm, Q0);
        quad::p1p1_to_p3(Pm, r);
        quad::to_cached(Q, Pm);
        tab[m * 4 + c] = Q;
      }
    }
  }
  __syncthreads();

  const fe *tA = w.tabA + 32ull * e0 + c;
  const fe *tR = mw.tabR + 32ull * e0 + c;
  auto adds_in = [](int wdx) { return 8 + (wdx <= 32 ? 8 : 0) + ((wdx & 1) ? 0 : 1); };
  auto fetch = [&](int wdx, int k, int &d) -> fe {
    if (k < 16) {
      const int jj = k & 7;
      const bool in = (in_sum >> jj) & 1;
      d = in ? dig[q][jj][k >> 3][wdx] : 0;
      const int a = d < 0 ? -d : d;
      return in ? (k < 8 ? tA : tR)[32 * jj + (a ? a - 1 : 0) * 4] : btab_q[c];
    }
    d = bdig[q][wdx >> 1];
    const int a = d < 0 ? -d : d;
    return btab_q[(a ? a - 1 : 0) * 4 + c];
  };
  fe idq, acc, r, nxt;
  int dn;
  quad::cached_identity(idq);
  quad::p3_identity(acc);
  nxt = fetch(63, 0, dn);
#pragma unroll 1
  for (int wdx = 63; wdx >= 0; wdx--) {
    if (wdx != 63) {
#pragma unroll
      for (int u = 0; u < 4; u++) {
        quad::dbl(r, acc);
        quad::p1p1_to_p3(acc, r);
      }
    }
    const int na = adds_in(wdx);
#pragma unroll 1
    for (int k = 0; k < na; k++) {
      fe ent = nxt;
      const int d = dn;
      if (k + 1 < na) {
        const int kn = (k + 1 >= 8 && wdx > 32) ? 16 : k + 1;
        nxt = fetch(wdx, kn, dn);
      } else if (wdx > 0) {
        nxt = fetch(wdx - 1, 0, dn);
      }
      fe_cmov(ent, idq, d == 0);
      quad::cached_cneg(ent, d < 0);
      quad::add(r, acc, ent);
      quad::p1p1_to_p3(acc, r);
    }
  }
  bool ok;
  if (SR) {
    fe id;
    quad::p3_identity(id);
    ok = quad::ristretto_equal(acc, id);
  } else {
    ok = quad::is_identity_times8(acc);
  }
  if (live && c == 0) mw.sub_ok[e0 >> kSubGroupLog2] = ok ? 1 : 0;
}

static size_t sort_smem(const MsmParams &p, uint32_t bs) {
  const size_t sort = bs * 9 + bs + 1 + 2 * (2 * p.m() + 1);
  const size_t merge = 6 * p.m() + 1 + 16 * merge_runs(p);
  return ((size_t)p.W * p.H + std::max(sort, merge)) * sizeof(uint32_t);
}

#ifdef TMV_CHECKS
__global__ void __launch_bounds__(256)
k_check_buckets(const uint32_t *count_ptr, uint32_t n, MsmWork mw, MsmParams p) {
  const uint32_t live_groups = (entry_count(count_ptr, n) + p.m() - 1) >> p.m_log2;
  const uint64_t nb = (uint64_t)live_groups * p.W * p.H;
  for (uint64_t b = blockIdx.x * (uint64_t)blockDim.x + threadIdx.x; b < nb; b += (uint64_t)gridDim.x * blockDim.x) {
    if (!mw.bk_cnt[b]) continue;
    const fe &z = mw.bk_sum[b].Z;
    bool zero = true;
#pragma unroll
    for (int k = 0; k < 10; k++) zero = zero && z.v[k] == 0;
    if (zero) atomicAdd(&g_buckets_unwritten, 1u);
  }
}
#endif

static std::atomic<uint32_t> g_compact_groups{kMsmCompactGroups};
void set_compact_groups(uint32_t g) { g_compact_groups = g ? g : kMsmCompactGroups; }
static bool compact_on(const MsmParams &p) { return p.groups >= g_compact_groups.load(std::memory_order_relaxed); }

static hipError_t launch_buckets(const uint32_t *count_ptr, uint32_t n, MsmWork mw, const MsmParams &p,
                                 hipStream_t stream, bool timed = true) {
  const uint64_t chunks = (uint64_t)p.groups * p.chunks_per_group();
  const uint32_t ablocks = (uint32_t)((chunks + 255) / 256), per_xcd = (ablocks + 7) / 8;
  hipError_t e;
#ifdef TMV_CHECKS
  if ((e = hipMemsetAsync(mw.bk_sum, 0, (size_t)p.groups * p.W * p.H * sizeof(ge_p3), stream)) != hipSuccess) return e;
#endif
  if (compact_on(p)) {
    hipLaunchKernelGGL(k_msm_chunk_scan, dim3(1), dim3(kScanBlock), 0, stream, count_ptr, n, mw, p);
    if ((e = hipGetLastError()) != hipSuccess) return e;
  } else {
    mw.chunk_end = nullptr;
  }
  void *tk = timed ? ktimer::begin(ktimer::kAccum, stream) : nullptr;
  if (p.L == 16)
    hipLaunchKernelGGL(k_msm_accum<16>, dim3(8 * per_xcd), dim3(256), 0, stream, count_ptr, n, mw, p);
  else
    hipLaunchKernelGGL(k_msm_accum<32>, dim3(8 * per_xcd), dim3(256), 0, stream, count_ptr, n, mw, p);
  if ((e = hipGetLastError()) != hipSuccess) return e;
  ktimer::end(tk, stream);
  const uint32_t jblocks = (uint32_t)std::min<uint64_t>(std::max<uint64_t>((chunks / 32 + 255) / 256, 1), 8192);
  hipLaunchKernelGGL(k_msm_join_list, dim3(jblocks), dim3(256), 0, stream, mw, p);
  if ((e = hipGetLastError()) != hipSuccess) return e;
#ifdef TMV_CHECKS
  hipLaunchKernelGGL(k_check_buckets, dim3(1024), dim3(256), 0, stream, count_ptr, n, mw, p);
  if ((e = hipGetLastError()) != hipSuccess) return e;
#endif
  const uint64_t parts = (uint64_t)p.groups * p.W * p.P;
  tk = timed ? ktimer::begin(ktimer::kWpart, stream) : nullptr;
  hipLaunchKernelGGL(k_msm_wpart, dim3((uint32_t)((parts + 255) / 256)), dim3(256), 0, stream, count_ptr, n, mw, p);
  if ((e = hipGetLastError()) != hipSuccess) return e;
  ktimer::end(tk, stream);
  if (p.P == 1) return hipSuccess;
  const uint64_t rows = (uint64_t)p.groups * p.W;
  hipLaunchKernelGGL(k_msm_wsum, dim3((uint32_t)((rows + 255) / 256)), dim3(256), 0, stream, count_ptr, n, mw, p);
  return hipGetLastError();
}

bool subcheck_enabled(uint32_t m_log2) { return m_log2 >= 8; }

bool read_checks(uint32_t out[3], bool reset) {
#ifdef TMV_CHECKS
  uint32_t v[3] = {0, 0, 0};
  if (hipDeviceSynchronize() != hipSuccess || hipMemcpyFromSymbol(&v[0], HIP_SYMBOL(g_joins_named), 4) != hipSuccess ||
      hipMemcpyFromSymbol(&v[1], HIP_SYMBOL(g_joins_done), 4) != hipSuccess ||
      hipMemcpyFromSymbol(&v[2], HIP_SYMBOL(g_buckets_unwritten), 4) != hipSuccess)
    return false;
  for (int k = 0; k < 3; k++) out[k] = v[k];
  if (reset) {
    const uint32_t z = 0;
    (void)hipMemcpyToSymbol(HIP_SYMBOL(g_joins_named), &z, 4);
    (void)hipMemcpyToSymbol(HIP_SYMBOL(g_joins_done), &z, 4);
    (void)hipMemcpyToSymbol(HIP_SYMBOL(g_buckets_unwritten), &z, 4);
  }
  return true;
#else
  (void)out;
  (void)reset;
  return false;
#endif
}

static uint32_t locate_min() {
  const char *e = getenv("TMV_LOCATE_MIN");
  return e ? (uint32_t)strtoul(e, nullptr, 10) : 400000u;
}

uint32_t locate_min_entries() { return locate_min(); }

bool locate_enabled(uint32_t n, const MsmParams &p) {
  const uint32_t lmin = locate_min();
  return lmin && n >= lmin && !p.sub && p.WL() <= p.W;
}

static std::atomic<int> g_key_merge{1};
void set_key_merge(int on) { g_key_merge = on ? 1 : 0; }
static bool key_merge_on() {
  const char *e = ab_knob("TMV_KEY_MERGE");
  return e ? atoi(e) != 0 : g_key_merge.load(std::memory_order_relaxed) != 0;
}

static Ed25519Work work_view(Ed25519Work w, uint64_t e0) {
  w.negA += 4 * e0;
  w.Rc += 4 * e0;
  w.k += 8 * e0;
  w.flags += 4 * e0;
  w.tabA += 64 * e0;
  w.hs_buf += 12 * e0;
  w.miss_list += e0;
  w.miss_count += e0 >> 5;
  return w;
}
static MsmWork msm_view(MsmWork mw, const MsmParams &p, uint32_t n, uint64_t g0) {
  const uint64_t e0 = g0 << p.m_log2, wh = (uint64_t)p.W * p.H;
  mw.pts += 2 * e0 * kNielsPer;
  mw.n_pts = (uint32_t)(2ull * n - 2 * e0);
  mw.ent_pt += g0 * p.cap;
  mw.ent_bk += g0 * p.cap;
  mw.bk_start += g0 * wh;
  mw.bk_cnt += g0 * wh;
  mw.bk_sum += g0 * wh;
  mw.part_first += g0 * p.chunks_per_group();
  mw.part_last += g0 * p.chunks_per_group();
  mw.join_b += g0 * p.chunks_per_group();
  mw.join_count += g0;
  mw.grp_chunks += g0;
  mw.chunk_end += g0;
  mw.wpart += g0 * p.W * 2ull * p.P;
  mw.wsum += g0 * p.W;
  mw.group_ok += g0;
  mw.sort_ovf += g0;
  if (mw.sub_ok) mw.sub_ok += (g0 << p.m_log2) / kSubGroup;
  if (mw.tabR) mw.tabR += 32 * e0;
  return mw;
}

template <bool SR, bool LOC>
static hipError_t launch_sort(const uint8_t *sig, const uint32_t *idx, const uint32_t *count_ptr, uint32_t n,
                              uint32_t e_base, const fe *btab_q, Ed25519Work w, MsmWork mw, const MsmParams &p,
                              const MsmSeed &seed, uint8_t *out, int aligned, hipStream_t stream) {
  mw.compact = compact_on(p) ? 1 : 0;
  if (p.m_log2 <= 8)
    hipLaunchKernelGGL((k_msm_sort<SR, false, 64, LOC>), dim3(p.groups), dim3(64), sort_smem(p, 64), stream, sig, idx,
                       count_ptr, n, w, mw, p, seed, btab_q, aligned, nullptr, nullptr, out, e_base);
  else
    hipLaunchKernelGGL((k_msm_sort<SR, false, kMsmSortBlock, LOC>), dim3(p.groups), dim3(kMsmSortBlock),
                       sort_smem(p, kMsmSortBlock), stream, sig, idx, count_ptr, n, w, mw, p, seed, btab_q, aligned,
                       nullptr, nullptr, out, e_base);
  return hipGetLastError();
}

template <bool SR>
static hipError_t launch_part(const uint8_t *pk, const uint8_t *sig, const uint8_t *msg, const uint32_t *msg_off,
                              const uint32_t *idx, const uint32_t *count_ptr, uint32_t n, uint32_t e_base,
                              const fe *btab_q, const strobe_t *prefix, Ed25519Work w, MsmWork mw,
                              const MsmParams &p, const MsmSeed &seed, uint8_t *out, int aligned,
                              hipStream_t stream) {
  w.niels = mw.pts;
  hipError_t e = launch_prep<SR>(pk, sig, msg, msg_off, idx, count_ptr, n, prefix, w, aligned, stream);
  if (e != hipSuccess) return e;
  if ((e = launch_sort<SR, false>(sig, idx, count_ptr, n, e_base, btab_q, w, mw, p, seed, out, aligned, stream)) !=
      hipSuccess)
    return e;
  return launch_buckets(count_ptr, n, mw, p, stream);
}

template <bool SR>
static hipError_t launch_tail_stages(const uint8_t *sig, const uint32_t *idx, const uint32_t *count_ptr, uint32_t n,
                                     const fe *btab_q, Ed25519Work w, MsmWork mw, const MsmParams &p,
                                     const MsmSeed &seed, uint8_t *out, int aligned, hipStream_t stream) {
  hipError_t e;
  const bool located = locate_enabled(n, p);
  const bool helped = !located && w.hs_buf;
  const uint32_t hblocks = (p.groups + 15) / 16;
  if (helped) {
    hipLaunchKernelGGL(k_msm_horner_helped<SR>, dim3(hblocks + (n + 63) / 64), dim3(64), 0, stream, count_ptr, n, mw,
                       p, w, hblocks);
    w.hs = w.hs_buf;
  } else {
    hipLaunchKernelGGL((k_msm_horner<SR, false>), dim3(hblocks), dim3(64), 0, stream, count_ptr, n, mw, p, nullptr,
                       0u);
  }
  if ((e = hipGetLastError()) != hipSuccess) return e;
  if (located) {
    if ((e = launch_sort<SR, true>(sig, idx, count_ptr, n, 0u, btab_q, w, mw, p, seed, nullptr, aligned, stream)) !=
        hipSuccess)
      return e;
    const uint32_t n_slots = p.groups << p.m_log2;
    if ((e = launch_buckets(mw.loc_count, n_slots, mw, p, stream, false)) != hipSuccess) return e;
    hipLaunchKernelGGL((k_msm_horner<SR, false, true>), dim3((p.groups + 15) / 16), dim3(64), 0, stream,
                       mw.loc_count, n_slots, mw, p, nullptr, 0u);
    if ((e = hipGetLastError()) != hipSuccess) return e;
    hipLaunchKernelGGL(k_loc_search<SR>, dim3(p.groups), dim3(64), 0, stream, count_ptr, n, mw, p);
    if ((e = hipGetLastError()) != hipSuccess) return e;
    return launch_quad_fallback<SR>(sig, idx, count_ptr, n, btab_q, w, mw.group_ok, p.m_log2, out, aligned, stream,
                                    nullptr, nullptr, nullptr, mw.fb_list, mw.fb_count);
  }
  const uint8_t *sub_ok = nullptr;
  if (p.sub) {
    const uint64_t subs = (uint64_t)p.groups << (p.m_log2 - kSubGroupLog2);
    hipLaunchKernelGGL(k_msm_subcheck<SR>, dim3((uint32_t)((subs + 15) / 16)), dim3(64), 0, stream, sig, idx,
                       count_ptr, n, w, mw, p, seed, btab_q, aligned, (const uint32_t *)mw.fail_list,
                       (const uint32_t *)mw.fail_count);
    if ((e = hipGetLastError()) != hipSuccess) return e;
    sub_ok = mw.sub_ok;
  }
  return launch_quad_fallback<SR>(sig, idx, count_ptr, n, btab_q, w, mw.group_ok, p.m_log2, out, aligned, stream,
                                  sub_ok, mw.fail_list, mw.fail_count);
}

__global__ void k_msm_count_groups(MsmWork mw, int located) {
  atomicAdd(&mw.ent_total[1], (unsigned long long)*mw.fail_count);
  if (located) {
    atomicAdd(&mw.ent_total[2], (unsigned long long)*mw.loc_found);
    atomicAdd(&mw.ent_total[3], (unsigned long long)*mw.fb_count);
  }
}

template <bool SR>
static hipError_t launch_tail(const uint8_t *sig, const uint32_t *idx, const uint32_t *count_ptr, uint32_t n,
                              const fe *btab_q, Ed25519Work w, MsmWork mw, const MsmParams &p, const MsmSeed &seed,
                              uint8_t *out, int aligned, hipStream_t stream) {
  hipError_t e = launch_tail_stages<SR>(sig, idx, count_ptr, n, btab_q, w, mw, p, seed, out, aligned, stream);
  if (e != hipSuccess || !mw.ent_total || !mw.fail_count) return e;
  hipLaunchKernelGGL(k_msm_count_groups, dim3(1), dim3(1), 0, stream, mw, locate_enabled(n, p) ? 1 : 0);
  return hipGetLastError();
}

template <bool SR>
static hipError_t launch_check(const uint8_t *pk, const uint8_t *sig, const uint8_t *msg, const uint32_t *msg_off,
                               const uint32_t *idx, const uint32_t *count_ptr, uint32_t n, const fe *btab_q,
                               const strobe_t *prefix, Ed25519Work w, MsmWork mw, const MsmParams &p,
                               const MsmSeed &seed, uint8_t *out, hipStream_t stream) {
  if (n == 0) return hipSuccess;
  const int aligned = ((((uintptr_t)pk) | ((uintptr_t)sig)) & 15) == 0;
  w.niels = mw.pts;
  mw.merge_pk = !SR && !count_ptr && key_merge_on() ? pk : nullptr;
  hipError_t e = launch_part<SR>(pk, sig, msg, msg_off, idx, count_ptr, n, 0u, btab_q, prefix, w, mw, p, seed, out,
                                 aligned, stream);
  if (e != hipSuccess) return e;
  return launch_tail<SR>(sig, idx, count_ptr, n, btab_q, w, mw, p, seed, out, aligned, stream);
}

hipError_t launch_batch_check_part(bool sr, const uint8_t *pk, const uint8_t *sig, const uint8_t *msg,
                                   const uint32_t *msg_off, uint32_t n, uint32_t e0, uint32_t e1, const fe *btab_q,
                                   const strobe_t *prefix, Ed25519Work w, MsmWork mw, const MsmParams &p,
                                   const MsmSeed &seed, uint8_t *out, hipStream_t stream) {
  if (e0 >= e1 || e1 > n || (e0 & (p.m() - 1)) || (e1 != n && (e1 & (p.m() - 1)))) return hipErrorInvalidValue;
  const int aligned = ((((uintptr_t)pk) | ((uintptr_t)sig)) & 15) == 0;
  const uint32_t g0 = e0 >> p.m_log2;
  MsmParams pp = p;
  pp.groups = ((e1 - e0) + p.m() - 1) >> p.m_log2;
  w.niels = mw.pts;
  const uint64_t E = e0;
  mw.merge_pk = !sr && key_merge_on() ? pk + 32 * E : nullptr;
  if (sr)
    return launch_part<true>(pk + 32 * E, sig + 64 * E, msg, msg_off + E, nullptr, nullptr, e1 - e0, e0, btab_q,
                             prefix, work_view(w, E), msm_view(mw, p, n, g0), pp, seed, out ? out + E : nullptr,
                             aligned, stream);
  return launch_part<false>(pk + 32 * E, sig + 64 * E, msg, msg_off + E, nullptr, nullptr, e1 - e0, e0, btab_q,
                            prefix, work_view(w, E), msm_view(mw, p, n, g0), pp, seed, out ? out + E : nullptr,
                            aligned, stream);
}

hipError_t launch_batch_check_tail(bool sr, const uint8_t *pk, const uint8_t *sig, uint32_t n, const fe *btab_q,
                                   Ed25519Work w, MsmWork mw, const MsmParams &p, const MsmSeed &seed,
                                   uint8_t *out, hipStream_t stream) {
  if (n == 0) return hipSuccess;
  const int aligned = ((((uintptr_t)pk) | ((uintptr_t)sig)) & 15) == 0;
  w.niels = mw.pts;
  mw.merge_pk = !sr && key_merge_on() ? pk : nullptr;
  if (sr) return launch_tail<true>(sig, nullptr, nullptr, n, btab_q, w, mw, p, seed, out, aligned, stream);
  return launch_tail<false>(sig, nullptr, nullptr, n, btab_q, w, mw, p, seed, out, aligned, stream);
}
// ... 26 lines not shown
}

__global__ void __launch_bounds__(kQuadBlock)
k_msm_items(KeyRuns runs, uint32_t n_items, MsmWork mw, KeyTable kt, const fe *__restrict__ bcomb) {
  constexpr int kItems = kQuadBlock / 4;
  __shared__ int8_t dig[kItems][64];
  if (blockIdx.x * kItems >= n_items) return;
  const int c = threadIdx.x & 3;
  const int q = threadIdx.x >> 2;
  const uint32_t raw = blockIdx.x * kItems + q;
  const bool live = raw < n_items;
  const uint32_t it = live ? raw : n_items - 1;
  const bool key = it < runs.n_runs;
  if (c == 0) {
    uint32_t sc[8];
    if (key) {
      uint32_t acc[9] = {0, 0, 0, 0, 0, 0, 0, 0, 0};
      for (uint32_t e = runs.lo[it]; e < runs.lo[it + 1]; e++) {
        const uint4 *wp = reinterpret_cast<const uint4 *>(mw.wscal + 8ull * e);
        const uint4 a = wp[0], b = wp[1];
        const uint32_t v[8] = {a.x, a.y, a.z, a.w, b.x, b.y, b.z, b.w};
        uint64_t cy = 0;
#pragma unroll
        for (int t = 0; t < 8; t++) {
          cy += (uint64_t)acc[t] + v[t];
          acc[t] = (uint32_t)cy;
          cy >>= 32;
        }
        acc[8] += (uint32_t)cy;
      }
      uint32_t x[16];
#pragma unroll
      for (int t = 0; t < 16; t++) x[t] = t < 9 ? acc[t] : 0;
      sc_reduce512(sc, x);
      recode16_store(&dig[q][0], sc, true);
    } else {
      const uint32_t *bs = mw.bscal + 8ull * (it - runs.n_runs);
#pragma unroll
      for (int t = 0; t < 8; t++) sc[t] = bs[t];
      recode256_store(&dig[q][0], sc);
    }
  }
  __syncthreads();
  fe acc, idq;
  quad::p3_identity(acc);
  quad::cached_identity(idq);
  if (key) {
    const fe *krow = kt.tab + (size_t)runs.slot[it] * kKeyRowsEntries * 4;
    comb_accumulate<64>(acc, idq, [&](int t, int &dsg) -> const fe * {
      dsg = dig[q][t];
      const int a = dsg < 0 ? -dsg : dsg;
      return krow + ((t * 8) + (a ? a - 1 : 0)) * 4 + c;
    });
  } else {
    comb_accumulate<32>(acc, idq, [&](int t, int &dsg) -> const fe * {
      dsg = dig[q][t];
      const int a = dsg < 0 ? -dsg : dsg;
      return bcomb + ((t * kBaseQuadEntries) + (a ? a - 1 : 0)) * 4 + c;
    });
  }
  if (live) mw.item_pt[4ull * it + c] = acc;
}

template <bool SR>
static hipError_t launch_km(const uint8_t *pk, const uint8_t *sig, const uint8_t *msg, const uint32_t *msg_off,
                            const uint32_t *key_slot, KeyRuns runs, uint32_t n, KeyTable kt, const fe *bcomb,
                            const strobe_t *prefix, Ed25519Work w, MsmWork mw, const MsmParams &p,
                            const MsmSeed &seed, uint8_t *out, hipStream_t stream) {
  if (n == 0) return hipSuccess;
  const int aligned = ((((uintptr_t)pk) | ((uintptr_t)sig)) & 15) == 0;
  w.niels = mw.pts;
  hipError_t e = launch_prep_cached<SR>(pk, sig, msg, msg_off, runs.order, n, prefix, w, aligned, stream);
  if (e != hipSuccess) return e;
  const size_t smem = sort_smem(p, kMsmSortBlock);
  mw.compact = compact_on(p) ? 1 : 0;
  hipLaunchKernelGGL((k_msm_sort<SR, true>), dim3(p.groups), dim3(kMsmSortBlock), smem, stream, sig, runs.order, nullptr,
                     n, w, mw, p, seed, nullptr, aligned, key_slot, kt.ok, nullptr, 0u);
  if ((e = hipGetLastError()) != hipSuccess) return e;
  if ((e = launch_buckets(nullptr, n, mw, p, stream)) != hipSuccess) return e;
  const uint32_t n_items = runs.n_runs + p.groups;
  hipLaunchKernelGGL(k_msm_items, dim3((n_items + 15) / 16), dim3(kQuadBlock), 0, stream, runs, n_items, mw, kt, bcomb);
  if ((e = hipGetLastError()) != hipSuccess) return e;
  hipLaunchKernelGGL((k_msm_horner<SR, true>), dim3((p.groups + 15) / 16), dim3(64), 0, stream, nullptr, n, mw, p,
                     runs.group_run0, runs.n_runs);
  if ((e = hipGetLastError()) != hipSuccess) return e;
  return launch_comb_fallback<SR>(sig, key_slot, runs.order, n, w, kt, bcomb, out, aligned, mw.group_ok, p.m_log2,
                                  stream);
}

hipError_t launch_key_merged_check(bool sr, const uint8_t *pk, const uint8_t *sig, const uint8_t *msg,
                                   const uint32_t *msg_off, const uint32_t *key_slot, KeyRuns runs, uint32_t n,
                                   KeyTable kt, const fe *bcomb, const strobe_t *prefix, Ed25519Work w, MsmWork mw,
                                   const MsmParams &p, const MsmSeed &seed, uint8_t *out, hipStream_t stream) {
  if (sr) return launch_km<true>(pk, sig, msg, msg_off, key_slot, runs, n, kt, bcomb, prefix, w, mw, p, seed, out, stream);
  return launch_km<false>(pk, sig, msg, msg_off, key_slot, runs, n, kt, bcomb, prefix, w, mw, p, seed, out, stream);
}

hipError_t launch_batch_check(bool sr, const uint8_t *pk, const uint8_t *sig, const uint8_t *msg,
                              const uint32_t *msg_off, const uint32_t *idx, const uint32_t *count_ptr, uint32_t n,
                              const fe *btab_q, const strobe_t *prefix, Ed25519Work w, MsmWork mw,
                              const MsmParams &p, const MsmSeed &seed, uint8_t *out, hipStream_t stream) {
  if (sr) return launch_check<true>(pk, sig, msg, msg_off, idx, count_ptr, n, btab_q, prefix, w, mw, p, seed, out, stream);
  return launch_check<false>(pk, sig, msg, msg_off, idx, count_ptr, n, btab_q, prefix, w, mw, p, seed, out, stream);
}

hipError_t launch_mixed_batch_check(const uint8_t *kind, const uint8_t *pk, const uint8_t *sig, const uint8_t *msg,
                                    const uint32_t *msg_off, uint32_t n, const fe *btab_q, const strobe_t *prefix,
                                    Ed25519Work w_ed, Ed25519Work w_sr, MsmWork m_ed, MsmWork m_sr,
                                    const MsmParams &p, const MsmParams &p_sr, const MsmSeed &seed_ed,
                                    const MsmSeed &seed_sr,
                                    uint32_t *counts, uint32_t *idx_ed, uint32_t *idx_sr, int8_t *status,
                                    hipStream_t stream, const KindStreams *ks) {
  if (n == 0) return hipSuccess;
  uint8_t *out = reinterpret_cast<uint8_t *>(status);
  hipError_t e = launch_partition(kind, n, counts, idx_ed, idx_sr, out, stream);
  if (e != hipSuccess) return e;
  hipStream_t s_sr = stream;
  if (ks && ks->helper && ks->fork && ks->join) {
    if ((e = hipEventRecord(ks->fork, stream)) != hipSuccess) return e;
    if ((e = hipStreamWaitEvent(ks->helper, ks->fork, 0)) != hipSuccess) return e;
    s_sr = ks->helper;
  }
  e = launch_check<true>(pk, sig, msg, msg_off, idx_sr, counts + 1, n, btab_q, prefix, w_sr, m_sr, p_sr, seed_sr,
                         out, s_sr);
  if (e != hipSuccess) return e;
  e = launch_check<false>(pk, sig, msg, msg_off, idx_ed, counts, n, btab_q, prefix, w_ed, m_ed, p, seed_ed, out,
                          stream);
  if (e != hipSuccess) return e;
  if (s_sr != stream) {
    if ((e = hipEventRecord(ks->join, s_sr)) != hipSuccess) return e;
    if ((e = hipStreamWaitEvent(stream, ks->join, 0)) != hipSuccess) return e;
  }
  return hipSuccess;
}

}
```

tendermint_amd/csrc/tmverify_runtime.cpp:

```cpp
#include <hip/hip_runtime.h>
#include <sys/random.h>

#include <cerrno>

#include <algorithm>
#include <array>
#include <atomic>
#include <chrono>
#include <cstdint>
#include <list>
#include <unordered_map>
#include <cstdlib>
#include <cstdio>
#include <cstring>
#include <functional>
#include <memory>
#include <condition_variable>
#include <mutex>
#include <string>
#include <thread>
#include <vector>

#include "../../include/tmverify.h"
#include "ed25519_core.h"
// ... 306 lines not shown
    const char *sc = getenv("TMV_STREAM_CHUNK");
    if (sc) g_stream_chunk = std::max<uint32_t>(2048, (uint32_t)strtoul(sc, nullptr, 10));
    const char *k = tmv::ab_knob("TMV_KERNEL");
    if (k && !strcmp(k, "quad")) g_kernel_override = 1;
    if (k && !strcmp(k, "single")) g_kernel_override = 0;
    const char *zc = tmv::ab_knob("TMV_ZERO_COPY");
    if (zc) g_zero_copy = atoi(zc);
    const char *ms = tmv::ab_knob("TMV_MIXED_STREAM");
    if (ms) g_mixed_stream = atoi(ms);
    const char *mxc = tmv::ab_knob("TMV_MIXED_CHUNK");
    if (mxc) g_mixed_chunk = std::max<uint32_t>(1, (uint32_t)strtoul(mxc, nullptr, 10));
    const char *hl = tmv::ab_knob("TMV_HOST_LANES");
    if (hl) g_host_lanes = std::min<uint32_t>(kLanes, std::max<uint32_t>(1, (uint32_t)strtoul(hl, nullptr, 10)));
    const char *mp = tmv::ab_knob("TMV_MSM_PARTS");
    if (mp) g_msm_parts = (uint32_t)strtoul(mp, nullptr, 10);
    const char *mc = tmv::ab_knob("TMV_MSM_CHUNK");
    if (mc) g_msm_chunk = (uint32_t)strtoul(mc, nullptr, 10);
    const char *st = tmv::ab_knob("TMV_STREAM");
    if (st) g_stream = atoi(st);
    const char *sg = tmv::ab_knob("TMV_SR_GROUP_LOG2");
    if (sg) g_sr_group_log2 = (uint32_t)strtoul(sg, nullptr, 10);
    const char *s2 = tmv::ab_knob("TMV_STREAM_TWO");
    if (s2) g_stream_two = atoi(s2);
    const char *rp = tmv::ab_knob("TMV_STREAM_RAMP");
    if (rp) g_stream_ramp = atoi(rp);
    const char *rg = tmv::ab_knob("TMV_REGISTER");
    if (rg) g_register = atoi(rg);
  });
}

hipStream_t context_stream(Device &d) {
  std::call_once(d.stream_once, [&] {
    (void)hipSetDevice(d.id);
    if (hipStreamCreateWithFlags(&d.stream, hipStreamNonBlocking) != hipSuccess) d.stream = nullptr;
  });
  return d.stream;
}

hipError_t wait_stream(Device &d, hipStream_t s) {
  read_env();
  hipError_t err = hipSuccess;
  const tmh::Poll r = tmh::poll_until([&] {
    const hipError_t e = hipStreamQuery(s);
    if (e == hipSuccess) return 0;
    if (e == hipErrorNotReady) return 1;
    err = e;
    return 2;
  }, g_timeout_ms);
  if (r == tmh::Poll::kTimeout) {
    d.faulted = true;
    set_error("device wait exceeded TMV_DEVICE_TIMEOUT_MS (" + std::to_string(g_timeout_ms) + " ms)");
    return hipErrorNotReady;
  }
  return err;
}
hipError_t wait_event(Device &d, hipEvent_t ev) {
  read_env();
  hipError_t err = hipSuccess;
  const tmh::Poll r = tmh::poll_until([&] {
    const hipError_t e = hipEventQuery(ev);
    if (e == hipSuccess) return 0;
    if (e == hipErrorNotReady) return 1;
    err = e;
    return 2;
  }, g_timeout_ms);
  if (r == tmh::Poll::kTimeout) {
    d.faulted = true;
    set_error("device wait exceeded TMV_DEVICE_TIMEOUT_MS (" + std::to_string(g_timeout_ms) + " ms)");
    return hipErrorNotReady;
  }
  return err;
}
int wait_rc(hipError_t e) { return e == hipErrorNotReady ? TMV_ERR_TIMEOUT : TMV_ERR_LAUNCH; }
int faulted_rc(Device &d) {
  set_error("device timed out earlier (TMV_ERR_TIMEOUT); open a new context");
  return TMV_ERR_TIMEOUT;
}

constexpr double kRunningSumWeight = 3.0;
static double running_sum_weight() {
  const char *e = tmv::ab_knob("TMV_RS_WEIGHT");
  return e ? atof(e) : kRunningSumWeight;
}
tmv::MsmParams msm_params(uint32_t n, uint32_t m_log2, uint32_t c, bool merged = false, bool ed_only = false,
                          int sub = -1) {
  const uint32_t lmin = tmv::locate_min_entries();
  if (m_log2 == 0) m_log2 = merged ? 8 : (ed_only && lmin && n >= lmin ? 7 : 6);
  m_log2 = std::max<uint32_t>(5, std::min<uint32_t>(10, m_log2));
  if (c == 0) {
    const double m = double(1u << m_log2), rsw = running_sum_weight();
    double best = 1e30;
    for (uint32_t cc = 4; cc <= 9; cc++) {
      const double W = (254 + cc - 1) / cc, WR = (129 + cc - 1) / cc, H = double(1u << (cc - 1));
      const double cost = merged ? m * WR + 2.2 * WR * H : m * (W + WR) + rsw * W * H;
      if (cost < best) { best = cost; c = cc; }
    }
  }
  c = std::max<uint32_t>(4, std::min<uint32_t>(9, c));
  tmv::MsmParams p = tmv::MsmParams::make(n, m_log2, c, merged);
  if (g_msm_chunk == 16 || g_msm_chunk == 32) p.L = g_msm_chunk;
  if (g_msm_parts && g_msm_parts <= p.H && !(g_msm_parts & (g_msm_parts - 1))) p.P = g_msm_parts;
  p.sub = merged ? 0 : (sub < 0 ? (tmv::subcheck_enabled(m_log2) ? 1 : 0) : (uint32_t)sub);
  return p;
}

struct EngineTimer {
  bool on = tmh::host_timing();
  std::chrono::steady_clock::time_point t = std::chrono::steady_clock::now();
  void mark(const char *what, uint32_t n) {
    if (!on) return;
    const auto now = std::chrono::steady_clock::now();
    fprintf(stderr, "[tmv_engine] %-8s %9.3f ms (n=%u)\n", what,
            std::chrono::duration<double, std::milli>(now - t).count(), n);
    t = now;
  }
};

struct Layout {
  size_t pk, sig, off, msg, total;
  Layout(uint32_t n, size_t msg_bytes) {
    pk = 0;
    sig = align16(pk + 32ull * n);
    off = align16(sig + 64ull * n);
    msg = align16(off + 4ull * (n + 1));
    total = align16(msg + std::max<size_t>(msg_bytes, 1));
  }
};

struct LaunchOpts {
  bool batch_eq = false;
  tmv::MsmParams p{};
  tmv::MsmParams p_ed{};
  tmv::MsmParams p_ed_streamed{};
  tmv::MsmSeed seed[2]{};
  int err = 0;
  bool stats = false;
};

std::atomic<int> g_rand_fault_err{0}, g_rand_fault_count{0};

int draw_weight_key(uint8_t key[32]) {
  size_t got = 0;
  while (got < 32) {
    ssize_t r;
    int fc = g_rand_fault_count.load();
    if (fc != 0) {
      if (fc > 0) g_rand_fault_count.fetch_sub(1);
      errno = g_rand_fault_err.load();
      r = -1;
    } else {
      r = getrandom(key + got, 32 - got, 0);
    }
    if (r > 0) {
      got += (size_t)r;
    } else if (r < 0 && errno == EINTR) {
      continue;
    } else {
      set_error(std::string("getrandom: ") + (r < 0 ? strerror(errno) : "no bytes"));
      return TMV_ERR_RANDOM;
    }
  }
  return 0;
}

}

struct tmv_ctx {
  std::vector<std::unique_ptr<Device>> devs;
  uint32_t msm_m_log2 = 0, msm_c = 0;
  int msm_sub = -1;
  bool fixed_seed = false, stats = false;
  uint8_t seed[32] = {0};
  std::atomic<uint64_t> launches{0};
  std::atomic<uint64_t> groups{0}, groups_failed{0}, subgroups{0}, subgroups_failed{0};
  std::atomic<uint64_t> m_calls{0}, m_sigs{0}, m_max{0}, m_beq{0}, m_host_sigs{0}, m_host_ns{0}, m_h2d{0}, m_d2h{0},
      m_located{0}, m_fallback{0};
  uint64_t khits_base = 0, kmiss_base = 0;
  std::mutex opt_mu;
  std::mutex host_mu;
  uint32_t host_inflight = 0;
  std::chrono::steady_clock::time_point host_t0;

  void host_enter() {
    std::lock_guard<std::mutex> lk(host_mu);
    if (host_inflight++ == 0) host_t0 = std::chrono::steady_clock::now();
// ... 52 lines not shown
  }
  return o;
}

static void collect_stats(tmv_ctx *ctx, Device &d, hipStream_t s) {
  auto it = d.ws.find(s);
  if (it == d.ws.end() || !it->second->group_ok[0]) return;
  Workspace &w = *it->second;
  uint32_t live[2] = {0, 0}, live_n[2] = {0, 0};
  if (w.counts) {
    uint32_t c[2];
    if (hipMemcpy(c, w.counts, sizeof(c), hipMemcpyDeviceToHost) != hipSuccess) return;
    for (int k = 0; k < 2; k++) {
      const uint32_t ml = k ? w.m_log2_sr : w.m_log2;
      live[k] = (c[k] + (1u << ml) - 1) >> ml;
      live_n[k] = c[k];
    }
  } else {
    live[0] = w.groups;
  }
  for (int k = 0; k < 2; k++) {
    if (!w.group_ok[k] || !live[k]) continue;
    const uint32_t mlog = k ? w.m_log2_sr : w.m_log2;
    std::vector<uint8_t> ok(live[k]);
    if (hipMemcpy(ok.data(), w.group_ok[k], live[k], hipMemcpyDeviceToHost) != hipSuccess) return;
    uint64_t failed = 0;
    for (uint8_t v : ok) failed += v ? 0 : 1;
    ctx->groups += live[k];
    ctx->groups_failed += failed;
    if (failed && w.loc[k]) {
      uint32_t lc[4];
      if (hipMemcpy(lc, w.loc[k], sizeof(lc), hipMemcpyDeviceToHost) != hipSuccess) return;
      ctx->m_fallback += lc[1];
      ctx->m_located += lc[2];
    } else if (failed && !w.sub_ok[k]) {
      const uint32_t m = 1u << mlog, nk = w.counts ? live_n[k] : w.n;
      for (uint32_t g = 0; g < live[k]; g++)
        if (!ok[g]) ctx->m_fallback += std::min<uint32_t>(m, nk - g * m);
    }
    if (!w.sub_ok[k] || !failed) continue;
    const uint32_t per = 1u << (mlog - tmv::kSubGroupLog2);
    std::vector<uint8_t> sub((size_t)live[k] * per);
    if (hipMemcpy(sub.data(), w.sub_ok[k], sub.size(), hipMemcpyDeviceToHost) != hipSuccess) return;
    uint64_t sfail = 0;
    for (uint32_t g = 0; g < live[k]; g++)
      if (!ok[g])
        for (uint32_t j = 0; j < per; j++) sfail += sub[(size_t)g * per + j] ? 0 : 1;
    ctx->subgroups += failed * per;
    ctx->subgroups_failed += sfail;
    for (uint32_t g = 0; g < live[k]; g++)
      if (!ok[g])
        for (uint32_t j = 0; j + 1 < per + 1; j += 2) {
          const bool bad = !sub[(size_t)g * per + j] || (j + 1 < per && !sub[(size_t)g * per + j + 1]);
          if (bad) ctx->m_fallback += 2 * tmv::kSubGroup;
        }
  }
  w.group_ok[0] = w.group_ok[1] = nullptr;
  w.sub_ok[0] = w.sub_ok[1] = nullptr;
  w.loc[0] = w.loc[1] = nullptr;
}

static int init_device(Device &d) {
  hipError_t e = hipSetDevice(d.id);
  if (e != hipSuccess) { set_error("hipSetDevice", e); return TMV_ERR_NO_DEVICE; }
  for (int l = 0; l < kLanes; l++) {
    e = hipStreamCreateWithFlags(&d.lane[l].stream, hipStreamNonBlocking);
    if (e != hipSuccess) { set_error("hipStreamCreate", e); return TMV_ERR_NO_DEVICE; }
  }
  std::vector<tmv::ge_precomp> table(tmv::kBaseTableRows * tmv::kBaseTableCols);
  tmv::build_base_table(table.data());
  const size_t bytes = table.size() * sizeof(tmv::ge_precomp);
  e = hipMalloc(&d.d_btable, bytes);
  if (e != hipSuccess) { set_error("hipMalloc(btable)", e); return TMV_ERR_NOMEM; }
  e = hipMemcpy(d.d_btable, table.data(), bytes, hipMemcpyHostToDevice);
  if (e != hipSuccess) { set_error("hipMemcpy(btable)", e); return TMV_ERR_NO_DEVICE; }
  {
    std::vector<uint32_t> gt(tmv::secp::kGTableWords);
    tmv::secp::build_g_table(gt.data());
    e = hipMalloc(&d.d_secp_gtab, gt.size() * sizeof(uint32_t));
    if (e != hipSuccess) { set_error("hipMalloc(secp gtab)", e); return TMV_ERR_NOMEM; }
    e = hipMemcpy(d.d_secp_gtab, gt.data(), gt.size() * sizeof(uint32_t), hipMemcpyHostToDevice);
    if (e != hipSuccess) { set_error("hipMemcpy(secp gtab)", e); return TMV_ERR_NO_DEVICE; }
  }
  std::vector<tmv::fe> bq(2 * 4 * tmv::kBaseQuadEntries);
  {
    tmv::ge_p3 B;
    tmv::ed25519_base_point(B);
    for (int h = 0; h < 2; h++) {
      if (h == 1)
        for (int d = 0; d < 128; d++) {
          tmv::ge_p1p1 t;
          tmv::ge_p3_dbl(t, B);
          tmv::ge_p1p1_to_p3(B, t);
        }
      tmv::ge_cached bc;
      tmv::ge_p3_to_cached(bc, B);
      tmv::ge_p3 P = B;
      for (int m = 0; m < tmv::kBaseQuadEntries; m++) {
        tmv::ge_precomp pc;
        tmv::ge_p3_to_precomp(pc, P);
        tmv::fe *o = &bq[4 * (h * tmv::kBaseQuadEntries + m)];
        o[0] = pc.ymx;
        o[1] = pc.ypx;
        o[2] = pc.xy2d;
        tmv::fe_one(o[3]);
        tmv::ge_p1p1 t;
        tmv::ge_add(t, P, bc);
        tmv::ge_p1p1_to_p3(P, t);
      }
    }
  }
  e = hipMalloc(&d.d_btab_q, bq.size() * sizeof(tmv::fe));
  if (e != hipSuccess) { set_error("hipMalloc(btab_q)", e); return TMV_ERR_NOMEM; }
  e = hipMemcpy(d.d_btab_q, bq.data(), bq.size() * sizeof(tmv::fe), hipMemcpyHostToDevice);
  if (e != hipSuccess) { set_error("hipMemcpy(btab_q)", e); return TMV_ERR_NO_DEVICE; }
  tmv::strobe_t prefix;
  tmv::sr25519_context_prefix(prefix);
  e = hipMalloc(&d.d_prefix, sizeof(prefix));
  if (e != hipSuccess) { set_error("hipMalloc(prefix)", e); return TMV_ERR_NOMEM; }
  e = hipMemcpy(d.d_prefix, &prefix, sizeof(prefix), hipMemcpyHostToDevice);
  if (e != hipSuccess) { set_error("hipMemcpy(prefix)", e); return TMV_ERR_NO_DEVICE; }
  e = hipEventCreateWithFlags(&d.work_done, hipEventDisableTiming);
  if (e != hipSuccess) { set_error("hipEventCreate", e); return TMV_ERR_NO_DEVICE; }
  {
    std::vector<tmv::fe> bc((size_t)32 * tmv::kBaseQuadEntries * 4);
    tmv::ge_p3 row, P;
    tmv::ed25519_base_point(row);
    for (int j = 0; j < 32; j++) {
      tmv::ge_cached rc;
      tmv::ge_p3_to_cached(rc, row);
      P = row;
      for (int m = 0; m < tmv::kBaseQuadEntries; m++) {
        tmv::ge_cached c;
        tmv::ge_p3_to_cached(c, P);
        tmv::fe *o = &bc[((size_t)j * tmv::kBaseQuadEntries + m) * 4];
        tmv::fe_carry(o[0], c.YmX);
        tmv::fe_carry(o[1], c.YpX);
        o[2] = c.T2d;
        o[3] = c.Z;
        tmv::ge_p1p1 t;
        tmv::ge_add(t, P, rc);
        tmv::ge_p1p1_to_p3(P, t);
      }
      for (int d = 0; d < 8; d++) {
        tmv::ge_p1p1 t;
        tmv::ge_p3_dbl(t, row);
        tmv::ge_p1p1_to_p3(row, t);
      }
    }
    e = hipMalloc(&d.d_bcomb, bc.size() * sizeof(tmv::fe));
    if (e != hipSuccess) { set_error("hipMalloc(bcomb)", e); return TMV_ERR_NOMEM; }
    e = hipMemcpy(d.d_bcomb, bc.data(), bc.size() * sizeof(tmv::fe), hipMemcpyHostToDevice);
    if (e != hipSuccess) { set_error("hipMemcpy(bcomb)", e); return TMV_ERR_NO_DEVICE; }
  }
  {
    std::vector<uint32_t> gc(tmv::secp::kCombWords);
    tmv::secp::ge g;
    tmv::secp::ge_generator(g);
    tmv::secp::build_comb(gc.data(), g);
    e = hipMalloc(&d.sk.d_gcomb, tmv::secp::kCombBytes);
    if (e != hipSuccess) { set_error("hipMalloc(secp gcomb)", e); return TMV_ERR_NOMEM; }
    e = hipMemcpy(d.sk.d_gcomb, gc.data(), tmv::secp::kCombBytes, hipMemcpyHostToDevice);
    if (e != hipSuccess) { set_error("hipMemcpy(secp gcomb)", e); return TMV_ERR_NO_DEVICE; }
  }
  const char *skc = getenv("TMV_SECP_KEY_CACHE_CAPACITY");
  d.sk.cap = skc ? (uint32_t)std::min<unsigned long>(strtoul(skc, nullptr, 10), 1ul << 20) : 4096u;
  const char *kc = getenv("TMV_KEY_CACHE_CAPACITY");
  d.kcap = kc ? (uint32_t)strtoul(kc, nullptr, 10) : 4096u;
  const char *ps = getenv("TMV_POINT_CACHE_SLOTS");
  d.pc_slots = tmv::pc_round_slots(ps ? strtoull(ps, nullptr, 10) : kPointCacheSlots);
  return 0;
}

static unsigned long long *entry_counter(Device &d) {
  if (!d.ent_tried) {
    d.ent_tried = true;
    void *p = nullptr;
    if (hipMalloc(&p, 32) != hipSuccess) {
      (void)hipGetLastError();
    } else if (hipMemset(p, 0, 32) != hipSuccess) {
      (void)hipGetLastError();
      (void)hipFree(p);
    } else {
      d.ent_total = static_cast<unsigned long long *>(p);
    }
  }
  return d.ent_total;
}

static std::atomic<int64_t> g_column_tile{-1};
static uint32_t column_tile() {
  const char *e = tmv::ab_knob("TMV_COLUMN_TILE");
  const int64_t v = e ? strtoll(e, nullptr, 10) : g_column_tile.load(std::memory_order_relaxed);
  return v < 0 ? tmv::kColumnTile : (uint32_t)std::min<int64_t>(v, tmv::kColumnMaxBatches);
}

static tmv::PointCache point_cache_view(Device &d, hipStream_t s) {
  if (!d.pc_tried && d.pc_slots) {
    d.pc_tried = true;
    const size_t tbytes = (size_t)d.pc_slots * tmv::kPcEntryWords * 4;
    void *p = nullptr;
    if (hipMalloc(&p, tbytes + 64) != hipSuccess) {
      (void)hipGetLastError();
    } else if (hipMemsetAsync(p, 0, tbytes + 64, s) != hipSuccess || hipStreamSynchronize(s) != hipSuccess) {
      (void)hipGetLastError();
      (void)hipFree(p);
    } else {
      d.pc.table = static_cast<tmv::pc_quad *>(p);
      d.pc.counters = reinterpret_cast<unsigned long long *>(static_cast<uint8_t *>(p) + tbytes);
      d.pc.bucket_mask = d.pc_slots / tmv::kPcWays - 1;
    }
  }
  tmv::PointCache v = d.pc;
  v.min_n = tmv::point_cache_min();
  return v;
}

static int resolve_keys(Device &d, bool sr, const uint8_t *pk, uint32_t n, uint32_t *slots_out, hipStream_t s) {
  if (d.kcap == 0) return 1;
  hipError_t e;
  if (!d.kt.tab) {
    if ((e = hipMalloc(&d.kt.tab, (size_t)d.kcap * tmv::KeyTable::bytes_per_key())) != hipSuccess) {
      set_error("hipMalloc(key table)", e);
      d.kt.tab = nullptr;
      return 1;
    }
    if ((e = hipMalloc(&d.kt.ok, d.kcap)) != hipSuccess) { set_error("hipMalloc(key ok)", e); return TMV_ERR_NOMEM; }
    d.kpos.resize(d.kcap);
    d.kslot_key.resize(d.kcap);
    d.kslot_epoch.assign(d.kcap, 0);
  }
  if (d.kindex.t.empty()) d.kindex.init(d.kcap);
  const uint64_t epoch = ++d.kepoch;
  std::vector<uint32_t> miss_idx;
  std::vector<uint32_t> miss_slot;
  constexpr uint32_t kParts = 16;
  const uint32_t parts = n >= 16384 ? kParts : 1;
  d.kseen.assign((size_t)parts * d.kcap, 0);
  uint32_t misses[kParts] = {0};
  std::vector<std::vector<uint32_t>> mb((size_t)parts * parts);
  auto key_part = [&](const uint8_t *k33) -> uint32_t {
    return parts == 1 ? 0u : (uint32_t)(KeyIndex::hash(k33) >> 58) & (kParts - 1);
  };
  auto lookup = [&](uint32_t part) {
    const uint32_t lo = (uint32_t)((uint64_t)n * part / parts), hi = (uint32_t)((uint64_t)n * (part + 1) / parts);
    uint8_t *seen = d.kseen.data() + (size_t)part * d.kcap;
    uint8_t key[33];
    key[0] = sr ? 1 : 0;
    const uint8_t *last_pk = nullptr;
    uint32_t last_slot = UINT32_MAX, miss = 0, last_q = 0;
    for (uint32_t i = lo; i < hi; i++) {
      const uint8_t *p = pk + 32ull * i;
      if (last_pk && std::memcmp(p, last_pk, 32) == 0) {
        slots_out[i] = last_slot;
        if (last_slot == UINT32_MAX) {
          miss++;
          mb[(size_t)part * parts + last_q].push_back(i);
        }
        continue;
      }
      std::memcpy(key + 1, p, 32);
      last_slot = slots_out[i] = d.kindex.find(key);
      last_pk = p;
// ... 413 lines not shown
  read_env();
  const bool quad = g_kernel_override == 1 || (g_kernel_override == -1 && n <= kQuadMax);
  hipError_t e;
  if (!quad) {
    e = tmv::launch_ed25519_verify(pk, sig, msg, off, n, d.d_btable, valid, s);
    if (e != hipSuccess) { set_error("k_ed25519_verify launch", e); return TMV_ERR_LAUNCH; }
    return 0;
  }
  int rc;
  Workspace *ws = reserve_work(d, n, false, s, &rc);
  if (!ws) return rc;
  tmv::Ed25519Work w = tmv::Ed25519Work::carve(ws->work.ptr, n);
  e = tmv::launch_ed25519_verify_quad(pk, sig, msg, off, n, d.d_btab_q, w, valid, s);
  if (e != hipSuccess) { set_error("k_ed25519_verify_quad launch", e); return TMV_ERR_LAUNCH; }
  (void)hipEventRecord(ws->done, s);
  return 0;
}

static uint32_t mixed_stream_chunk(size_t free_bytes);

extern "C" {

int tmv_kernel_timing(tmv_ctx *ctx, int enable) {
  if (!ctx) { set_error("null context"); return TMV_ERR_ARG; }
  tmv::ktimer::set(enable != 0);
  return 0;
}

int tmv_kernel_timing_read(tmv_ctx *ctx, const char *kernel, double *total_ms, uint64_t *launches) {
  if (!ctx || !kernel || !total_ms || !launches) { set_error("null argument"); return TMV_ERR_ARG; }
  tmv::ktimer::Kernel k;
  if (!strcmp(kernel, "k_msm_accum")) k = tmv::ktimer::kAccum;
  else if (!strcmp(kernel, "k_msm_wpart")) k = tmv::ktimer::kWpart;
  else if (!strcmp(kernel, "k_prep_fused")) k = tmv::ktimer::kPrep;
  else if (!strcmp(kernel, "k_secp_prep")) k = tmv::ktimer::kSecpPrep;
  else if (!strcmp(kernel, "k_secp_verify")) k = tmv::ktimer::kSecpVerify;
  else if (!strcmp(kernel, "k_secp_key_table")) k = tmv::ktimer::kSecpKeyTable;
  else if (!strcmp(kernel, "k_secp_prep_cached")) k = tmv::ktimer::kSecpPrepCached;
  else if (!strcmp(kernel, "k_secp_verify_comb")) k = tmv::ktimer::kSecpVerifyComb;
  else if (!strcmp(kernel, "k_merkle_leaves_long")) k = tmv::ktimer::kMerkleLeavesLong;
  else if (!strcmp(kernel, "k_merkle_tree_levels")) k = tmv::ktimer::kMerkleTreeLevels;
  else if (!strcmp(kernel, "k_merkle_aunts")) k = tmv::ktimer::kMerkleAunts;
  else if (!strcmp(kernel, "k_merkle_verify_proofs")) k = tmv::ktimer::kMerkleVerify;
  else if (!strcmp(kernel, "k_merkle_leaves")) k = tmv::ktimer::kMerkleLeaves;
  else if (!strcmp(kernel, "k_commit_leaves")) k = tmv::ktimer::kCommitLeaves;
  else if (!strcmp(kernel, "k_vote_ext_signbytes")) k = tmv::ktimer::kVoteExtSignbytes;
  else if (!strcmp(kernel, "k_merkle_digests_long")) k = tmv::ktimer::kMerkleDigestsLong;
  else if (!strcmp(kernel, "k_merkle_value_ops")) k = tmv::ktimer::kMerkleValueOps;
  else if (!strcmp(kernel, "k_result_leaves")) k = tmv::ktimer::kResultLeaves;
  else { set_error("unknown timed kernel"); return TMV_ERR_ARG; }
  *total_ms = 0;
  *launches = 0;
  const int e = tmv::ktimer::read(k, total_ms, launches);
  if (e) { set_error("hipEventElapsedTime", (hipError_t)e); return TMV_ERR_LAUNCH; }
  return 0;
}

const char *tmv_last_error(void) { return g_last_error.c_str(); }
void tmv_internal_set_error(const char *msg) { g_last_error = msg ? msg : ""; }

void tmv_internal_random_fault(int err, int count) {
  g_rand_fault_err = err;
  g_rand_fault_count = count;
}
int tmv_internal_option(const char *name, int64_t value) {
  if (name && !strcmp(name, "half_scalars")) {
    tmv::set_half_scalar_mode((int)value);
    return 0;
  }
  if (name && !strcmp(name, "point_cache_min")) {
    tmv::set_point_cache_min(value < 0 ? 0u : (uint32_t)value);
    return 0;
  }
  if (name && !strcmp(name, "column_tile")) {
    g_column_tile = value;
    return 0;
  }
  if (name && !strcmp(name, "compact_groups")) {
    tmv::set_compact_groups(value < 0 ? 0u : (uint32_t)value);
    return 0;
  }
  if (name && !strcmp(name, "key_merge")) {
    tmv::set_key_merge(value != 0);
    return 0;
  }
  set_error("unknown internal option");
  return TMV_ERR_ARG;
}
int tmv_internal_checks(uint32_t *out3, int reset) {
  if (!out3) { set_error("null argument"); return TMV_ERR_ARG; }
  if (!tmv::read_checks(out3, reset != 0)) {
    set_error("not a TMV_CHECKS build, or the device read failed");
    return TMV_ERR_ARG;
  }
  return 0;
}
int64_t tmv_internal_mixed_stream_chunk(uint64_t free_bytes) {
  read_env();
  return mixed_stream_chunk((size_t)free_bytes);
}
int tmv_internal_draw_key(uint8_t *out32) {
  if (!out32) { set_error("null argument"); return TMV_ERR_ARG; }
  return draw_weight_key(out32);
}

tmv_ctx *tmv_open(uint32_t device_mask) { return tmv_open_logical(device_mask, 1); }

tmv_ctx *tmv_open_logical(uint32_t device_mask, int logical) {
  release_leaked_pins();
  int count = 0;
  hipError_t e = hipGetDeviceCount(&count);
  if (e != hipSuccess || count <= 0) {
    set_error(e != hipSuccess ? std::string("hipGetDeviceCount: ") + hipGetErrorString(e)
                              : std::string("no HIP device visible"));
    return nullptr;
  }
  logical = std::max(1, std::min(8, logical));
  if (logical > 1)
    fprintf(stderr, "tmverify: TEST AID tmv_open_logical: every GPU opened as %d logical devices\n", logical);
  auto ctx = std::make_unique<tmv_ctx>();
  for (int i = 0; i < count && i < 32; i++) {
    if (device_mask != 0 && !(device_mask & (1u << i))) continue;
    for (int k = 0; k < logical; k++) {
      auto d = std::make_unique<Device>();
      d->id = i;
      if (init_device(*d) != 0) {
        tmv_close(ctx.release());
        return nullptr;
      }
      ctx->devs.push_back(std::move(d));
    }
  }
  if (ctx->devs.empty()) {
    set_error("device_mask selects no visible device");
    return nullptr;
  }
  return ctx.release();
}

void tmv_close(tmv_ctx *ctx) {
  if (!ctx) return;
  for (auto &d : ctx->devs) {
    if (d->faulted) continue;
    (void)hipSetDevice(d->id);
    for (HostLane &l : d->lane) {
      if (l.stream) (void)hipStreamSynchronize(l.stream);
      if (l.copy) (void)hipStreamSynchronize(l.copy);
    }
  }
  release_leaked_pins();
  for (auto &d : ctx->devs) {
    (void)hipSetDevice(d->id);
    if (d->faulted) continue;
    if (d->stream) (void)hipStreamSynchronize(d->stream);
    for (HostLane &l : d->lane) {
      if (l.stream) (void)hipStreamSynchronize(l.stream);
      if (l.copy) (void)hipStreamSynchronize(l.copy);
      for (hipEvent_t ev : l.part_ready) (void)hipEventDestroy(ev);
      l.part_ready.clear();
      for (hipEvent_t ev : l.part_split) (void)hipEventDestroy(ev);
      l.part_split.clear();
      if (l.copy) (void)hipStreamDestroy(l.copy);
      l.copy = nullptr;
      if (l.helper) (void)hipStreamSynchronize(l.helper);
      if (l.helper) (void)hipStreamDestroy(l.helper);
      if (l.join) (void)hipEventDestroy(l.join);
// ... 647 lines not shown

int tmv_set_batch_options(tmv_ctx *ctx, uint32_t group_log2, uint32_t window_bits, const uint8_t *seed32,
                          uint32_t opt_flags) {
  if (!ctx) { set_error("null context"); return TMV_ERR_ARG; }
  if ((group_log2 && (group_log2 < 5 || group_log2 > 10)) || (window_bits && (window_bits < 4 || window_bits > 9))) {
    set_error("group_log2 must be 0 or 5..10, window_bits 0 or 4..9");
    return TMV_ERR_ARG;
  }
  std::lock_guard<std::mutex> lk(ctx->opt_mu);
  ctx->msm_m_log2 = group_log2;
  ctx->msm_c = window_bits;
  ctx->fixed_seed = seed32 != nullptr;
  if (seed32) std::memcpy(ctx->seed, seed32, 32);
  ctx->stats = (opt_flags & TMV_BATCHOPT_STATS) != 0;
  ctx->msm_sub = (opt_flags & TMV_BATCHOPT_SUBCHECK_ON) ? 1 : (opt_flags & TMV_BATCHOPT_SUBCHECK_OFF) ? 0 : -1;
  return 0;
}

int tmv_batch_stats(tmv_ctx *ctx, uint64_t *groups, uint64_t *groups_failed) {
  if (!ctx) return TMV_ERR_ARG;
  if (groups) *groups = ctx->groups.load();
  if (groups_failed) *groups_failed = ctx->groups_failed.load();
  return 0;
}

int tmv_subgroup_stats(tmv_ctx *ctx, uint64_t *subgroups, uint64_t *subgroups_failed) {
  if (!ctx) return TMV_ERR_ARG;
  if (subgroups) *subgroups = ctx->subgroups.load();
  if (subgroups_failed) *subgroups_failed = ctx->subgroups_failed.load();
  return 0;
}

int tmv_key_cache_stats(tmv_ctx *ctx, uint64_t *hits, uint64_t *misses, uint32_t *used, uint32_t *capacity) {
  if (!ctx) return TMV_ERR_ARG;
  uint64_t h = 0, m = 0;
  uint32_t u = 0, c = 0;
  for (auto &d : ctx->devs) {
    std::lock_guard<std::mutex> lk(d->mu);
    h += d->khits; m += d->kmisses; u += (uint32_t)d->kindex.size(); c += d->kcap;
  }
  if (hits) *hits = h;
  if (misses) *misses = m;
  if (used) *used = u;
  if (capacity) *capacity = c;
  return 0;
}

int tmv_point_cache_stats(tmv_ctx *ctx, uint64_t *hits, uint64_t *misses, uint32_t *slots) {
  if (!ctx) return TMV_ERR_ARG;
  uint64_t h = 0, m = 0;
  uint32_t c = 0;
  for (auto &d : ctx->devs) {
    std::lock_guard<std::mutex> lk(d->mu);
    c += d->pc_slots;
    if (!d->pc.table) continue;
    unsigned long long v[2];
    hipError_t e = hipSetDevice(d->id);
    if (e == hipSuccess) e = hipMemcpy(v, d->pc.counters, sizeof(v), hipMemcpyDeviceToHost);
    if (e != hipSuccess) { set_error("point cache counters", e); return TMV_ERR_NO_DEVICE; }
    h += v[0]; m += v[1];
  }
  if (hits) *hits = h;
  if (misses) *misses = m;
  if (slots) *slots = c;
  return 0;
}

int tmv_bucket_entry_stats(tmv_ctx *ctx, uint64_t *entries) {
  if (!ctx) return TMV_ERR_ARG;
  uint64_t t = 0;
  for (auto &d : ctx->devs) {
    std::lock_guard<std::mutex> lk(d->mu);
    if (!d->ent_total) continue;
    unsigned long long v = 0;
    hipError_t e = hipSetDevice(d->id);
    if (e == hipSuccess) e = hipMemcpy(&v, d->ent_total, sizeof(v), hipMemcpyDeviceToHost);
    if (e != hipSuccess) { set_error("bucket entry counter", e); return TMV_ERR_NO_DEVICE; }
    t += v;
  }
  if (entries) *entries = t;
  return 0;
}

int tmv_group_fail_stats(tmv_ctx *ctx, uint64_t *groups_failed, uint64_t *groups_located, uint64_t *fallback_entries) {
  if (!ctx) return TMV_ERR_ARG;
  uint64_t t[3] = {0, 0, 0};
  for (auto &d : ctx->devs) {
    std::lock_guard<std::mutex> lk(d->mu);
    if (!d->ent_total) continue;
    unsigned long long v[4] = {0, 0, 0, 0};
    hipError_t e = hipSetDevice(d->id);
    if (e == hipSuccess) e = hipMemcpy(v, d->ent_total, sizeof(v), hipMemcpyDeviceToHost);
    if (e != hipSuccess) { set_error("group counters", e); return TMV_ERR_NO_DEVICE; }
    for (int k = 0; k < 3; k++) t[k] += v[k + 1];
  }
  if (groups_failed) *groups_failed = t[0];
  if (groups_located) *groups_located = t[1];
  if (fallback_entries) *fallback_entries = t[2];
  return 0;
}

#ifdef TMV_CHECKS
int tmv_internal_point_cache_read(tmv_ctx *ctx, uint8_t *out, uint64_t bytes) {
  if (!ctx || !out || ctx->devs.empty()) return TMV_ERR_ARG;
  Device &d = *ctx->devs[0];
  std::lock_guard<std::mutex> lk(d.mu);
  if (!d.pc.table || bytes != (uint64_t)d.pc_slots * 64) return TMV_ERR_ARG;
  if (hipSetDevice(d.id) != hipSuccess || hipDeviceSynchronize() != hipSuccess ||
      hipMemcpy(out, d.pc.table, bytes, hipMemcpyDeviceToHost) != hipSuccess)
    return TMV_ERR_NO_DEVICE;
  return 0;
}
int tmv_internal_point_cache_write(tmv_ctx *ctx, const uint8_t *in, uint64_t bytes) {
  if (!ctx || !in || ctx->devs.empty()) return TMV_ERR_ARG;
  Device &d = *ctx->devs[0];
  std::lock_guard<std::mutex> lk(d.mu);
  if (!d.pc.table || bytes != (uint64_t)d.pc_slots * 64) return TMV_ERR_ARG;
  if (hipSetDevice(d.id) != hipSuccess || hipDeviceSynchronize() != hipSuccess ||
      hipMemcpy(d.pc.table, in, bytes, hipMemcpyHostToDevice) != hipSuccess || hipDeviceSynchronize() != hipSuccess)
    return TMV_ERR_NO_DEVICE;
  return 0;
}
#endif

int tmv_metrics_read(tmv_ctx *ctx, tmv_metrics *out) {
  if (!ctx || !out) { set_error("null argument"); return TMV_ERR_ARG; }
  std::memset(out, 0, sizeof(*out));
  out->calls = ctx->m_calls;
  out->signatures = ctx->m_sigs;
  out->max_batch = ctx->m_max;
  out->batch_eq_signatures = ctx->m_beq;
  out->host_signatures = ctx->m_host_sigs;
  out->host_seconds = (double)ctx->m_host_ns.load() * 1e-9;
  out->h2d_bytes = ctx->m_h2d;
  out->d2h_bytes = ctx->m_d2h;
  out->groups = ctx->groups;
  out->groups_failed = ctx->groups_failed;
  out->located_groups = ctx->m_located;
  out->fallback_signatures = ctx->m_fallback;
  uint64_t h = 0, m = 0;
  for (auto &d : ctx->devs) {
    std::lock_guard<std::mutex> lk(d->mu);
    h += d->khits;
    m += d->kmisses;
  }
  out->key_cache_hits = h - ctx->khits_base;
  out->key_cache_misses = m - ctx->kmiss_base;
  return 0;
}

int tmv_metrics_reset(tmv_ctx *ctx) {
  if (!ctx) { set_error("null context"); return TMV_ERR_ARG; }
  for (auto *a : {&ctx->m_calls, &ctx->m_sigs, &ctx->m_max, &ctx->m_beq, &ctx->m_host_sigs, &ctx->m_host_ns,
                  &ctx->m_h2d, &ctx->m_d2h, &ctx->m_located, &ctx->m_fallback, &ctx->groups, &ctx->groups_failed,
                  &ctx->subgroups, &ctx->subgroups_failed})
    a->store(0);
  uint64_t h = 0, m = 0;
  for (auto &d : ctx->devs) {
    std::lock_guard<std::mutex> lk(d->mu);
    h += d->khits;
    m += d->kmisses;
  }
  ctx->khits_base = h;
  ctx->kmiss_base = m;
  return 0;
}
// ... 414 lines not shown
```

Measured before the change: 232.2 million.

## Split MSM windows for sparse groups using precomputed shifted high points

Adds a window-splitting mode to the ed25519 batch MSM. In groups with few nonzero scalars (leaders), each point's high-half digits are redirected to a precomputed 2^(c*Ws)-shifted copy of the point, so only about half as many windows are processed. A new kernel computes the shifted points by repeated doubling, and the base point gets a host-precomputed shifted entry. This is meant to cut bucket and Horner work per group, at the cost of extra doublings, inversions, workspace and sort-kernel complexity. It is enabled by default only when groups >= 4096 with P==1, or when split_groups is forced to 1.

Result: faster. 247.9 million (median of 6 runs) (+6.8%).

```diff
diff --git a/__graft_entry__.py b/__graft_entry__.py
--- a/__graft_entry__.py
+++ b/__graft_entry__.py
@@ -17,6 +17,7 @@
     subprocess.run(["make", "-s", "-C", os.path.join(REPO, "tests", "native", "merkle")], check=True)
     subprocess.run(["make", "-s", "-C", os.path.join(REPO, "tests", "native", "pcache")], check=True)
     subprocess.run(["make", "-s", "-C", os.path.join(REPO, "tests", "native", "colorder")], check=True)
+    subprocess.run(["make", "-s", "-C", os.path.join(REPO, "tests", "native", "split")], check=True)
     subprocess.run(["make", "-s", "-C", os.path.join(REPO, "tests", "native", "blocks")], check=True)
     subprocess.run(["make", "-s", "-C", os.path.join(REPO, "tests", "native", "voteext")], check=True)
     subprocess.run(["make", "-s", "-C", os.path.join(REPO, "tests", "native", "proofops")], check=True)
diff --git a/include/tmverify.h b/include/tmverify.h
--- a/include/tmverify.h
+++ b/include/tmverify.h
@@ -115,6 +115,8 @@
 
 int tmv_group_fail_stats(tmv_ctx *ctx, uint64_t *groups_failed, uint64_t *groups_located, uint64_t *fallback_entries);
 
+int tmv_split_stats(tmv_ctx *ctx, uint64_t *groups_split, uint64_t *high_points);
+
 typedef struct tmv_metrics {
   uint64_t calls;
   uint64_t signatures;
diff --git a/tendermint_amd/_native.py b/tendermint_amd/_native.py
--- a/tendermint_amd/_native.py
+++ b/tendermint_amd/_native.py
@@ -47,6 +47,7 @@
     "tmv_secp256k1_key_cache_stats",
     "tmv_verify_mixed_batch", "tmv_ed25519_verify_batch_device", "tmv_verify_mixed_batch_device",
     "tmv_verify_batch_ex", "tmv_key_cache_stats", "tmv_point_cache_stats", "tmv_bucket_entry_stats", "tmv_group_fail_stats",
+    "tmv_split_stats",
     "tmv_set_batch_options", "tmv_batch_stats",
     "tmv_subgroup_stats", "tmv_validator_set_hashes",
     "tmv_verify_mixed_batch_ex", "tmv_verify_batch_device_ex", "tmv_verify_batches_device",
@@ -174,6 +175,7 @@
                                             ctypes.POINTER(ctypes.c_uint32)]
         L.tmv_bucket_entry_stats.argtypes = [vp, ctypes.POINTER(ctypes.c_uint64)]
         L.tmv_group_fail_stats.argtypes = [vp] + [ctypes.POINTER(ctypes.c_uint64)] * 3
+        L.tmv_split_stats.argtypes = [vp] + [ctypes.POINTER(ctypes.c_uint64)] * 2
         L.tmv_set_batch_options.argtypes = [vp, ctypes.c_uint32, ctypes.c_uint32, u8p, ctypes.c_uint32]
         L.tmv_batch_stats.argtypes = [vp, ctypes.POINTER(ctypes.c_uint64), ctypes.POINTER(ctypes.c_uint64)]
         L.tmv_kernel_timing.argtypes = [vp, ctypes.c_int]
@@ -672,6 +674,11 @@
                     "tmv_group_fail_stats")
         return {"failed": f.value, "located": l.value, "fallback_entries": e.value}
 
+    def split_stats(self) -> dict:
+        g, h = ctypes.c_uint64(), ctypes.c_uint64()
+        self._check(self._lib.tmv_split_stats(self._h, ctypes.byref(g), ctypes.byref(h)), "tmv_split_stats")
+        return {"groups_split": g.value, "high_points": h.value}
+
     def metrics(self) -> dict:
         m = Metrics()
         self._check(self._lib.tmv_metrics_read(self._h, ctypes.byref(m)), "tmv_metrics_read")
diff --git a/tendermint_amd/csrc/msm.h b/tendermint_amd/csrc/msm.h
--- a/tendermint_amd/csrc/msm.h
+++ b/tendermint_amd/csrc/msm.h
@@ -1,6 +1,8 @@
 #pragma once
+#include <stddef.h>
 #include <stdint.h>
 #include "curve25519.h"
+#include "split.h"
 
 namespace tmv {
 
@@ -8,6 +10,8 @@
 constexpr int kMsmChunkMax = 32;
 constexpr uint32_t kMsmEmpty = 0xffffffffu;
 constexpr uint32_t kMsmCompactGroups = 2048;
+constexpr uint32_t kMsmSplitGroups = 4096;
+constexpr uint32_t kMsmSplitMax = 8;
 constexpr int kMsmSortBlock = 256;
 constexpr uint32_t kSubGroupLog2 = 3;
 constexpr uint32_t kSubGroup = 1u << kSubGroupLog2;
@@ -52,6 +56,11 @@
   uint32_t L;
   uint32_t merged;
   uint32_t sub;
+  uint32_t Ws;
+  uint32_t Wa;
+  uint32_t Wl;
+  uint32_t split_max;
+  uint32_t split;
 
   TMV_HD uint32_t m() const { return 1u << m_log2; }
   TMV_HD uint32_t WL() const { return (129 + m_log2 + c - 1) / c; }
@@ -84,6 +93,11 @@
       if (chain < best) { best = chain; p.P = P; }
     }
     if ((uint64_t)p.groups * p.W >= kMsmWideRows) p.P = 1;
+    p.Ws = split_windows(p.W);
+    p.Wa = p.Ws > p.WR ? p.Ws : p.WR;
+    p.Wl = p.Ws > p.WL() ? p.Ws : p.WL();
+    p.split_max = 0;
+    p.split = 0;
     return p;
   }
 };
@@ -117,6 +131,12 @@
   uint32_t *loc_found;
   uint32_t *fb_list;
   const uint8_t *merge_pk;
+  uint8_t *grp_split;
+  uint32_t *hi_of;
+  uint32_t *hi_list;
+  uint32_t *uns_list;
+  uint32_t *split_cnt;
+  uint32_t g_base;
   unsigned long long *ent_total;
   uint32_t *wscal;
   uint32_t *bscal;
@@ -124,15 +144,19 @@
 
   static size_t max_items(uint32_t n, const MsmParams &p) { return (size_t)n + 2ull * p.groups; }
 
+  static size_t point_slots(uint32_t n, const MsmParams &p) {
+    return 2ull * n + 1 + (p.split ? 1 + (size_t)p.groups * p.split_max : 0);
+  }
   static size_t bytes(uint32_t n, const MsmParams &p) {
     const size_t G = p.groups, bk = (size_t)G * p.buckets_per_group(), ent = (size_t)G * p.cap;
     const size_t chunks = ent / p.L;
-    size_t b = (2ull * n + 1) * kNielsPer * sizeof(niels_pt) + 8 * ent + 8 * bk + bk * sizeof(ge_p3) +
+    size_t b = point_slots(n, p) * kNielsPer * sizeof(niels_pt) + 8 * ent + 8 * bk + bk * sizeof(ge_p3) +
                2 * chunks * sizeof(ge_p3) + 4 * chunks + G * p.W * (2ull * p.wpart_slots() + 1) * sizeof(ge_p3) + G + 2 * G +
                18 * 16 + 4 * G + 8 * G + 32;
     if (p.merged) b += 32ull * n + 32 * G + max_items(n, p) * 4 * sizeof(fe);
     else b += 16 + 4 * G + (G << p.m_log2) / kSubGroup + 16 + (size_t)n * 32 * sizeof(fe) + 3 * 16 +
               G * 8 * sizeof(fe) + 16 + 4ull * n + 2 * 16 + 4 * G + 2 * 16 + G * 4 * sizeof(fe) + 16;
+    if (p.split) b += 2 * G + 4ull * n + 8 * G * p.split_max + 4 * G + 8 * G + 5 * 16;
     return b;
   }
   static MsmWork carve(void *base, uint32_t n, const MsmParams &p) {
@@ -142,7 +166,7 @@
     const size_t chunks = ent / p.L;
     MsmWork w;
     size_t o = 0;
-    w.pts = reinterpret_cast<niels_pt *>(b + o); o = up(o + (2ull * n + 1) * kNielsPer * sizeof(niels_pt));
+    w.pts = reinterpret_cast<niels_pt *>(b + o); o = up(o + point_slots(n, p) * kNielsPer * sizeof(niels_pt));
     w.ent_pt = reinterpret_cast<uint32_t *>(b + o); o = up(o + 4 * ent);
     w.ent_bk = reinterpret_cast<uint32_t *>(b + o); o = up(o + 4 * ent);
     w.bk_start = reinterpret_cast<uint32_t *>(b + o); o = up(o + 4 * bk);
@@ -160,6 +184,9 @@
     w.sort_ovf = b + o; o = up(o + 2 * G);
     w.n_pts = 2 * n;
     w.merge_pk = nullptr;
+    w.grp_split = nullptr;
+    w.hi_of = w.hi_list = w.uns_list = w.split_cnt = nullptr;
+    w.g_base = 0;
     w.compact = 0;
     w.ent_total = nullptr;
     w.wscal = w.bscal = nullptr;
@@ -186,6 +213,13 @@
       w.bscal = reinterpret_cast<uint32_t *>(b + o); o = up(o + 32 * G);
       w.item_pt = reinterpret_cast<fe *>(b + o);
     }
+    if (p.split) {
+      w.grp_split = b + o; o = up(o + 2 * G);
+      w.hi_of = reinterpret_cast<uint32_t *>(b + o); o = up(o + 4ull * n);
+      w.hi_list = reinterpret_cast<uint32_t *>(b + o); o = up(o + 8 * G * p.split_max);
+      w.uns_list = reinterpret_cast<uint32_t *>(b + o); o = up(o + 4 * G);
+      w.split_cnt = reinterpret_cast<uint32_t *>(b + o); o = up(o + 8 * G);
+    }
     return w;
   }
 };
diff --git a/tendermint_amd/csrc/msm_kernels.hip b/tendermint_amd/csrc/msm_kernels.hip
--- a/tendermint_amd/csrc/msm_kernels.hip
+++ b/tendermint_amd/csrc/msm_kernels.hip
@@ -150,6 +150,13 @@
 
 TMV_HD uint32_t merge_runs(const MsmParams &p) { return p.m() / 2 < 256u ? p.m() / 2 : 256u; }
 
+constexpr uint32_t kSplitWords = 40;
+TMV_HD uint32_t sort_words(const MsmParams &p, uint32_t bs) {
+  const uint32_t sort = bs * 9 + bs + 1 + 2 * (2 * p.m() + 1);
+  const uint32_t merge = 6 * p.m() + 1 + 16 * merge_runs(p);
+  return p.W * p.H + (sort > merge ? sort : merge);
+}
+
 __device__ __forceinline__ void p3_dbl(ge_p3 &a) {
   ge_p1p1 r;
   ge_p3_dbl(r, a);
@@ -158,7 +165,7 @@
 
 }
 
-template <bool SR, bool KM, int BS = kMsmSortBlock, bool LOC = false>
+template <bool SR, bool KM, int BS = kMsmSortBlock, bool LOC = false, bool SPLIT = false>
 __global__ void __launch_bounds__(BS)
 k_msm_sort(const uint8_t *__restrict__ sig, const uint32_t *__restrict__ idx, const uint32_t *count_ptr, uint32_t n,
            Ed25519Work w, MsmWork mw, MsmParams p, MsmSeed seed, const fe *__restrict__ btab_q, int aligned,
@@ -188,6 +195,13 @@
     bp.xy2d = btab_q[2];
     bp.pad[0] = bp.pad[1] = 0;
     niels_store(mw.pts, mw.n_pts, bp);
+    if constexpr (SPLIT) {
+      const fe *bh = btab_q + 4 * (2 * kBaseQuadEntries + (p.c - 4));
+      bp.ymx = bh[0];
+      bp.ypx = bh[1];
+      bp.xy2d = bh[2];
+      niels_store(mw.pts, mw.n_pts + 1, bp);
+    }
     if (mw.fail_count) *mw.fail_count = 0;
   }
   if (e0 >= cnt) return;
@@ -420,13 +434,92 @@
     }
   }
 
+  bool split_g = false;
+  uint32_t hi_pt[R];
+  int carry_hi[R], carry_bhi = 0;
+  uint32_t *lmask = smem + sort_words(p, BS), *lbad = lmask + 32, *lbase = lmask + 33;
+  if constexpr (SPLIT) {
+    bool lead[R];
+#pragma unroll
+    for (int r = 0; r < R; r++) {
+      hi_pt[r] = 0;
+      carry_hi[r] = 0;
+      uint32_t nz = 0;
+#pragma unroll
+      for (int t = 0; t < 8; t++) nz |= wv[r][t];
+      lead[r] = live[r] && nz != 0;
+    }
+    if (tid < 34) lmask[tid] = 0;
+    __syncthreads();
+#pragma unroll
+    for (int r = 0; r < R; r++) {
+      const uint32_t j = tid + r * BS;
+      if (lead[r]) atomicOr(&lmask[j >> 5], 1u << (j & 31));
+    }
+    __syncthreads();
+    uint32_t leaders = 0;
+    for (uint32_t k = 0; k < (p.m() + 31) / 32; k++) leaders += __popc(lmask[k]);
+    split_g = LOC ? mw.grp_split[g] != 0 : leaders <= p.split_max;
+    if (tid == 0) {
+      mw.grp_split[(LOC ? p.groups : 0) + slot] = split_g ? 1 : 0;
+      if (!split_g) {
+        mw.uns_list[atomicAdd(&mw.split_cnt[1], 1u)] = slot;
+      } else if (!LOC) {
+        *lbase = atomicAdd(&mw.split_cnt[0], leaders);
+        if (mw.ent_total) {
+          atomicAdd(&mw.ent_total[4], 1ull);
+          atomicAdd(&mw.ent_total[5], (unsigned long long)leaders);
+        }
+      }
+    }
+    if (split_g) {
+      if (!LOC) __syncthreads();
+#pragma unroll
+      for (int r = 0; r < R; r++) {
+        if (!live[r]) continue;
+        const uint32_t j = tid + r * BS, e = e0 + j;
+        uint32_t gslot = kMsmEmpty;
+        if (LOC) {
+          if (lead[r]) {
+            gslot = mw.hi_of[e];
+            if (gslot == kMsmEmpty) atomicOr(lbad, 1u);
+          }
+        } else {
+          if (lead[r]) {
+            uint32_t rank = __popc(lmask[j >> 5] & ((1u << (j & 31)) - 1));
+            for (uint32_t k = 0; k < (j >> 5); k++) rank += __popc(lmask[k]);
+            gslot = (mw.g_base + g) * p.split_max + rank;
+            mw.hi_list[2 * (*lbase + rank)] = e;
+            mw.hi_list[2 * (*lbase + rank) + 1] = gslot;
+          }
+          mw.hi_of[e] = gslot;
+        }
+        hi_pt[r] = mw.n_pts + 2 + gslot;
+      }
+    }
+  }
+  auto count_split = [&](const uint32_t *s, int &cy) {
+    DigitReader<8> rd;
+    rd.init(s);
+    for (uint32_t w = 0; w < p.W; w++) {
+      if (w == p.Ws) cy = rd.carry;
+      const int d = rd.next(p.c, w + 1 == p.W);
+      if (d != 0) atomicAdd(&hist[p.bucket(split_slot(w, p.Ws, split_g).window, (uint32_t)((d < 0 ? -d : d) - 1))], 1u);
+    }
+  };
+
 #pragma unroll
   for (int r = 0; r < R; r++) {
     if (!live[r]) continue;
     for_each_digit<ZW>(z[r], WRz, p, [&](uint32_t bk, bool) { atomicAdd(&hist[bk], 1u); });
-    if (!KM) for_each_digit<8>(wv[r], p.W, p, [&](uint32_t bk, bool) { atomicAdd(&hist[bk], 1u); });
-  }
-  if (!KM && tid == 0) for_each_digit<8>(bsc, p.W, p, [&](uint32_t bk, bool) { atomicAdd(&hist[bk], 1u); });
+    if constexpr (SPLIT) count_split(wv[r], carry_hi[r]);
+    else if (!KM) for_each_digit<8>(wv[r], p.W, p, [&](uint32_t bk, bool) { atomicAdd(&hist[bk], 1u); });
+  }
+  if constexpr (SPLIT) {
+    if (tid == 0) count_split(bsc, carry_bhi);
+  } else {
+    if (!KM && tid == 0) for_each_digit<8>(bsc, p.W, p, [&](uint32_t bk, bool) { atomicAdd(&hist[bk], 1u); });
+  }
   __syncthreads();
 
   const uint32_t seg = (WH + BS - 1) / BS;
@@ -447,7 +540,7 @@
   __syncthreads();
   const uint32_t gbase = slot * p.cap;
   const uint32_t bbase = slot * WH;
-  const bool ovf = scan[BS] > p.cap;
+  const bool ovf = scan[BS] > p.cap || (SPLIT && *lbad != 0);
   if (tid == 0) mw.sort_ovf[(LOC ? p.groups : 0) + slot] = ovf ? 1 : 0;
   if (tid == 0 && !ovf && mw.ent_total) atomicAdd(mw.ent_total, (unsigned long long)scan[BS]);
   if (tid == 0) mw.grp_chunks[slot] = ovf ? 0u : (scan[BS] + p.L - 1) / p.L;
@@ -476,6 +569,69 @@
   const uint32_t wcap = 2 * p.m() + 1;
   uint32_t *st_pt = scan + BS + 1, *st_bk = st_pt + wcap;
   DigitReader<ZW> rz[R];
+  const uint32_t total = scan[BS];
+  if constexpr (SPLIT) {
+    DigitReader<5> rlo[R], rblo;
+    DigitReader<4> rhi[R], rbhi;
+    const uint32_t sh = p.c * p.Ws;
+    auto high_half = [&](DigitReader<4> &rd, const uint32_t *s, int cy) {
+      uint32_t t[9], h[4];
+#pragma unroll
+      for (int k = 0; k < 8; k++) t[k] = s[k];
+      t[8] = 0;
+      for (uint32_t i = 0; i < (sh >> 5); i++) {
+#pragma unroll
+        for (int k = 0; k < 8; k++) t[k] = t[k + 1];
+      }
+#pragma unroll
+      for (int k = 0; k < 4; k++) h[k] = (uint32_t)((((uint64_t)t[k + 1] << 32) | t[k]) >> (sh & 31));
+      rd.init(h);
+      rd.carry = cy;
+    };
+#pragma unroll
+    for (int r = 0; r < R; r++) {
+      rz[r].init(z[r]);
+      rlo[r].init(wv[r]);
+      high_half(rhi[r], wv[r], carry_hi[r]);
+    }
+    rblo.init(bsc);
+    high_half(rbhi, bsc, carry_bhi);
+    const uint32_t Wg = split_g ? (LOC ? p.Wl : p.Wa) : p.W;
+    for (uint32_t w = 0; w < Wg; w++) {
+      const uint32_t wbeg = hist[p.bucket(w, 0)];
+      const uint32_t wend = w + 1 < p.W ? hist[p.bucket(w + 1, 0)] : total;
+      __syncthreads();
+      auto put = [&](int d, uint32_t pt) {
+        if (d == 0) return;
+        const uint32_t bk = p.bucket(w, (uint32_t)((d < 0 ? -d : d) - 1));
+        const uint32_t pos = atomicAdd(&hist[bk], 1u) - wbeg;
+        st_pt[pos] = (pt << 1) | (d < 0 ? 1u : 0u);
+        st_bk[pos] = bbase + bk;
+      };
+      const uint32_t wh = split_g ? w + p.Ws : w;
+      const bool lo_on = w < p.Ws, hi_on = wh >= p.Ws && wh < p.W;
+#pragma unroll
+      for (int r = 0; r < R; r++) {
+        if (!live[r]) continue;
+        const uint32_t e = e0 + tid + r * BS;
+        if (w < WRz) put(rz[r].next(p.c, w + 1 == WRz), 2 * e);
+        if (lo_on) put(rlo[r].next(p.c, false), 2 * e + 1);
+        if (hi_on) put(rhi[r].next(p.c, wh + 1 == p.W), split_g ? hi_pt[r] : 2 * e + 1);
+      }
+      if (tid == 0) {
+        if (lo_on) put(rblo.next(p.c, false), mw.n_pts);
+        if (hi_on) put(rbhi.next(p.c, wh + 1 == p.W), split_g ? mw.n_pts + 1 : mw.n_pts);
+      }
+      __syncthreads();
+      for (uint32_t i = tid; i < wend - wbeg; i += BS) {
+        ent_pt[wbeg + i] = st_pt[i];
+        ent_bk[wbeg + i] = st_bk[i];
+      }
+    }
+    const uint32_t pad_end = mw.compact ? min(p.cap, (total + p.L - 1) / p.L * p.L) : p.cap;
+    for (uint32_t t = total + tid; t < pad_end; t += BS) ent_bk[t] = kMsmEmpty;
+    return;
+  }
   DigitReader<8> rw[R], rb;
 #pragma unroll
   for (int r = 0; r < R; r++) {
@@ -483,7 +639,6 @@
     rw[r].init(wv[r]);
   }
   rb.init(bsc);
-  const uint32_t total = scan[BS];
   for (uint32_t w = 0; w < p.W; w++) {
     const uint32_t wbeg = hist[p.bucket(w, 0)];
     const uint32_t wend = w + 1 < p.W ? hist[p.bucket(w + 1, 0)] : total;
@@ -528,6 +683,44 @@
   }
   const uint32_t pad_end = mw.compact ? min(p.cap, (total + p.L - 1) / p.L * p.L) : p.cap;
   for (uint32_t t = total + tid; t < pad_end; t += BS) ent_bk[t] = kMsmEmpty;
+}
+
+constexpr int kHiBlock = 256;
+__global__ void __launch_bounds__(kHiBlock)
+k_msm_hi_points(Ed25519Work w, MsmWork mw, MsmParams p) {
+  constexpr uint32_t kPts = kHiBlock / 4;
+  __shared__ fe zs[kPts];
+  const uint32_t cnt = mw.split_cnt[0];
+  if (blockIdx.x * kPts >= cnt) return;
+  const uint32_t q = threadIdx.x >> 2, raw = blockIdx.x * kPts + q;
+  const bool live = raw < cnt;
+  const uint32_t i = live ? raw : cnt - 1;
+  const int c = (int)(threadIdx.x & 3);
+  const uint32_t e = mw.hi_list[2 * i], gslot = mw.hi_list[2 * i + 1];
+  fe acc = w.negA[4ull * e + c], r;
+  for (uint32_t d = 0; d < p.c * p.Ws; d++) {
+    quad::dbl(r, acc);
+    quad::p1p1_to_p3(acc, r);
+  }
+  if (c == 2) zs[q] = acc;
+  __syncthreads();
+  if (threadIdx.x < kPts) {
+    fe zi;
+    fe_invert(zi, zs[threadIdx.x]);
+    zs[threadIdx.x] = zi;
+  }
+  __syncthreads();
+  fe a, x, y, t, u;
+  fe_mul(a, acc, zs[q]);
+  quad::fe_dpp<quad::qp(0, 0, 0, 0)>(x, a);
+  quad::fe_dpp<quad::qp(1, 1, 1, 1)>(y, a);
+  quad::fe_dpp<quad::qp(3, 3, 3, 3)>(t, a);
+  niels_pt np;
+  fe_add(u, y, x); fe_carry(np.ypx, u);
+  fe_sub(u, y, x); fe_carry(np.ymx, u);
+  fe_mul(np.xy2d, t, consts::d2());
+  np.pad[0] = np.pad[1] = 0;
+  if (live && c == 0) niels_store(mw.pts, (uint64_t)mw.n_pts + 2 + gslot, np);
 }
 
 #ifdef TMV_CHECKS
@@ -729,12 +922,31 @@
 }
 
 __global__ void __launch_bounds__(256)
-k_msm_wpart(const uint32_t *count_ptr, uint32_t n, MsmWork mw, MsmParams p) {
-  const uint32_t t = blockIdx.x * blockDim.x + threadIdx.x;
+k_msm_wpart(const uint32_t *count_ptr, uint32_t n, MsmWork mw, MsmParams p, const uint8_t *__restrict__ gsplit,
+            uint32_t wa) {
+  uint32_t t = blockIdx.x * blockDim.x + threadIdx.x;
   const uint32_t per_group = p.W * p.P;
-  const uint32_t g = t / per_group;
+  uint32_t g, r;
+  if (gsplit) {
+    const uint32_t b1 = (p.groups * wa + blockDim.x - 1) / blockDim.x;
+    if (blockIdx.x < b1) {
+      g = t / wa;
+      r = t - g * wa;
+    } else {
+      const uint32_t t2 = (blockIdx.x - b1) * blockDim.x + threadIdx.x, rest = p.W - wa;
+      const uint32_t u = t2 / rest;
+      if (u >= mw.split_cnt[1]) return;
+      g = mw.uns_list[u];
+      r = wa + (t2 - u * rest);
+    }
+    t = g * per_group + r;
+  } else {
+    g = t / per_group;
+    r = t - g * per_group;
+  }
   if (g >= p.groups || (g << p.m_log2) >= entry_count(count_ptr, n)) return;
-  const uint32_t r = t - g * per_group, wdx = r / p.P, part = r % p.P;
+  const uint32_t wdx = r / p.P, part = r % p.P;
+  const uint32_t top = gsplit && gsplit[g] ? wa - 1 : p.W - 1;
   const uint32_t s = p.H / p.P;
   ge_p3 U, T;
   bool u_set = false, t_set = false;
@@ -785,7 +997,7 @@
     mw.wpart[2ull * t] = T;
     mw.wpart[2ull * t + 1] = U;
   } else {
-    store_window_sum(&mw.wpart[2ull * t], T, wdx == p.W - 1);
+    store_window_sum(&mw.wpart[2ull * t], T, wdx == top);
   }
 }
 
@@ -814,7 +1026,8 @@
 template <bool SR, bool KM, bool LOC>
 __device__ __forceinline__ void horner_block(uint32_t bx, const uint32_t *count_ptr, uint32_t n, MsmWork mw,
                                              const MsmParams &p, const uint32_t *__restrict__ group_run0,
-                                             uint32_t n_runs) {
+                                             uint32_t n_runs, const uint8_t *__restrict__ gsplit = nullptr,
+                                             uint32_t wa = 0) {
   const uint32_t live_groups = (entry_count(count_ptr, n) + p.m() - 1) >> p.m_log2;
   if (bx * 16 >= live_groups) return;
   const uint32_t raw = bx * 16 + (threadIdx.x >> 2);
@@ -823,9 +1036,10 @@
   const int c = (int)(threadIdx.x & 3);
   const uint32_t st = p.P == 1 ? 2 : 1;
   const ge_p3 *S = p.P == 1 ? mw.wpart + 2ull * g * p.W : mw.wsum + (size_t)g * p.W;
-  fe acc = reinterpret_cast<const fe *>(&S[st * (p.W - 1)])[c];
+  const uint32_t top = gsplit && gsplit[g] ? wa - 1 : p.W - 1;
+  fe acc = reinterpret_cast<const fe *>(&S[st * top])[c];
   fe r, q, qc;
-  for (int wI = (int)p.W - 2; wI >= 0; wI--) {
+  for (int wI = (int)top - 1; wI >= 0; wI--) {
     qc = reinterpret_cast<const fe *>(&S[st * wI])[c];
     for (uint32_t d = 0; d < p.c; d++) {
       quad::dbl(r, acc);
@@ -871,8 +1085,8 @@
 template <bool SR, bool KM, bool LOC = false>
 __global__ void __launch_bounds__(64)
 k_msm_horner(const uint32_t *count_ptr, uint32_t n, MsmWork mw, MsmParams p, const uint32_t *__restrict__ group_run0,
-             uint32_t n_runs) {
-  horner_block<SR, KM, LOC>(blockIdx.x, count_ptr, n, mw, p, group_run0, n_runs);
+             uint32_t n_runs, const uint8_t *__restrict__ gsplit, uint32_t wa) {
+  horner_block<SR, KM, LOC>(blockIdx.x, count_ptr, n, mw, p, group_run0, n_runs, gsplit, wa);
 }
 
 template <bool SR>
@@ -1145,10 +1359,8 @@
   if (live && c == 0) mw.sub_ok[e0 >> kSubGroupLog2] = ok ? 1 : 0;
 }
 
-static size_t sort_smem(const MsmParams &p, uint32_t bs) {
-  const size_t sort = bs * 9 + bs + 1 + 2 * (2 * p.m() + 1);
-  const size_t merge = 6 * p.m() + 1 + 16 * merge_runs(p);
-  return ((size_t)p.W * p.H + std::max(sort, merge)) * sizeof(uint32_t);
+static size_t sort_smem(const MsmParams &p, uint32_t bs, bool split = false) {
+  return ((size_t)sort_words(p, bs) + (split ? kSplitWords : 0)) * sizeof(uint32_t);
 }
 
 #ifdef TMV_CHECKS
@@ -1167,12 +1379,14 @@
 }
 #endif
 
+static bool split_on(const MsmWork &mw, const MsmParams &p) { return p.split && mw.merge_pk && mw.grp_split; }
+
 static std::atomic<uint32_t> g_compact_groups{kMsmCompactGroups};
 void set_compact_groups(uint32_t g) { g_compact_groups = g ? g : kMsmCompactGroups; }
 static bool compact_on(const MsmParams &p) { return p.groups >= g_compact_groups.load(std::memory_order_relaxed); }
 
 static hipError_t launch_buckets(const uint32_t *count_ptr, uint32_t n, MsmWork mw, const MsmParams &p,
-                                 hipStream_t stream, bool timed = true) {
+                                 hipStream_t stream, bool timed = true, bool loc = false) {
   const uint64_t chunks = (uint64_t)p.groups * p.chunks_per_group();
   const uint32_t ablocks = (uint32_t)((chunks + 255) / 256), per_xcd = (ablocks + 7) / 8;
   hipError_t e;
@@ -1201,7 +1415,15 @@
 #endif
   const uint64_t parts = (uint64_t)p.groups * p.W * p.P;
   tk = timed ? ktimer::begin(ktimer::kWpart, stream) : nullptr;
-  hipLaunchKernelGGL(k_msm_wpart, dim3((uint32_t)((parts + 255) / 256)), dim3(256), 0, stream, count_ptr, n, mw, p);
+  if (split_on(mw, p)) {
+    const uint32_t wa = loc ? p.Wl : p.Wa;
+    const uint64_t b1 = ((uint64_t)p.groups * wa + 255) / 256, b2 = ((uint64_t)p.groups * (p.W - wa) + 255) / 256;
+    hipLaunchKernelGGL(k_msm_wpart, dim3((uint32_t)(b1 + b2)), dim3(256), 0, stream, count_ptr, n, mw, p,
+                       (const uint8_t *)mw.grp_split + (loc ? p.groups : 0), wa);
+  } else {
+    hipLaunchKernelGGL(k_msm_wpart, dim3((uint32_t)((parts + 255) / 256)), dim3(256), 0, stream, count_ptr, n, mw, p,
+                       (const uint8_t *)nullptr, 0u);
+  }
   if ((e = hipGetLastError()) != hipSuccess) return e;
   ktimer::end(tk, stream);
   if (p.P == 1) return hipSuccess;
@@ -1283,6 +1505,14 @@
   mw.wsum += g0 * p.W;
   mw.group_ok += g0;
   mw.sort_ovf += g0;
+  if (mw.grp_split) {
+    mw.grp_split += g0;
+    mw.hi_of += e0;
+    mw.hi_list += 2 * g0 * p.split_max;
+    mw.uns_list += g0;
+    mw.split_cnt += 2 * g0;
+    mw.g_base = (uint32_t)g0;
+  }
   if (mw.sub_ok) mw.sub_ok += (g0 << p.m_log2) / kSubGroup;
   if (mw.tabR) mw.tabR += 32 * e0;
   return mw;
@@ -1293,6 +1523,21 @@
                               uint32_t e_base, const fe *btab_q, Ed25519Work w, MsmWork mw, const MsmParams &p,
                               const MsmSeed &seed, uint8_t *out, int aligned, hipStream_t stream) {
   mw.compact = compact_on(p) ? 1 : 0;
+  if constexpr (!SR) {
+    if (split_on(mw, p)) {
+      hipError_t e = hipMemsetAsync(mw.split_cnt, 0, 2 * sizeof(uint32_t), stream);
+      if (e != hipSuccess) return e;
+      if (p.m_log2 <= 8)
+        hipLaunchKernelGGL((k_msm_sort<false, false, 64, LOC, true>), dim3(p.groups), dim3(64), sort_smem(p, 64, true),
+                           stream, sig, idx, count_ptr, n, w, mw, p, seed, btab_q, aligned, nullptr, nullptr, out,
+                           e_base);
+      else
+        hipLaunchKernelGGL((k_msm_sort<false, false, kMsmSortBlock, LOC, true>), dim3(p.groups), dim3(kMsmSortBlock),
+                           sort_smem(p, kMsmSortBlock, true), stream, sig, idx, count_ptr, n, w, mw, p, seed, btab_q,
+                           aligned, nullptr, nullptr, out, e_base);
+      return hipGetLastError();
+    }
+  }
   if (p.m_log2 <= 8)
     hipLaunchKernelGGL((k_msm_sort<SR, false, 64, LOC>), dim3(p.groups), dim3(64), sort_smem(p, 64), stream, sig, idx,
                        count_ptr, n, w, mw, p, seed, btab_q, aligned, nullptr, nullptr, out, e_base);
@@ -1315,6 +1560,11 @@
   if ((e = launch_sort<SR, false>(sig, idx, count_ptr, n, e_base, btab_q, w, mw, p, seed, out, aligned, stream)) !=
       hipSuccess)
     return e;
+  if (split_on(mw, p)) {
+    const uint64_t hb = ((uint64_t)p.groups * p.split_max + kHiBlock / 4 - 1) / (kHiBlock / 4);
+    hipLaunchKernelGGL(k_msm_hi_points, dim3((uint32_t)hb), dim3(kHiBlock), 0, stream, w, mw, p);
+    if ((e = hipGetLastError()) != hipSuccess) return e;
+  }
   return launch_buckets(count_ptr, n, mw, p, stream);
 }
 
@@ -1324,7 +1574,9 @@
                                      const MsmSeed &seed, uint8_t *out, int aligned, hipStream_t stream) {
   hipError_t e;
   const bool located = locate_enabled(n, p);
-  const bool helped = !located && w.hs_buf;
+  const bool split = split_on(mw, p);
+  const uint8_t *gsplit = split ? mw.grp_split : nullptr;
+  const bool helped = !located && w.hs_buf && !split;
   const uint32_t hblocks = (p.groups + 15) / 16;
   if (helped) {
     hipLaunchKernelGGL(k_msm_horner_helped<SR>, dim3(hblocks + (n + 63) / 64), dim3(64), 0, stream, count_ptr, n, mw,
@@ -1332,7 +1584,7 @@
     w.hs = w.hs_buf;
   } else {
     hipLaunchKernelGGL((k_msm_horner<SR, false>), dim3(hblocks), dim3(64), 0, stream, count_ptr, n, mw, p, nullptr,
-                       0u);
+                       0u, gsplit, p.Wa);
   }
   if ((e = hipGetLastError()) != hipSuccess) return e;
   if (located) {
@@ -1340,9 +1592,9 @@
         hipSuccess)
       return e;
     const uint32_t n_slots = p.groups << p.m_log2;
-    if ((e = launch_buckets(mw.loc_count, n_slots, mw, p, stream, false)) != hipSuccess) return e;
+    if ((e = launch_buckets(mw.loc_count, n_slots, mw, p, stream, false, true)) != hipSuccess) return e;
     hipLaunchKernelGGL((k_msm_horner<SR, false, true>), dim3((p.groups + 15) / 16), dim3(64), 0, stream,
-                       mw.loc_count, n_slots, mw, p, nullptr, 0u);
+                       mw.loc_count, n_slots, mw, p, nullptr, 0u, split ? mw.grp_split + p.groups : nullptr, p.Wl);
     if ((e = hipGetLastError()) != hipSuccess) return e;
     hipLaunchKernelGGL(k_loc_search<SR>, dim3(p.groups), dim3(64), 0, stream, count_ptr, n, mw, p);
     if ((e = hipGetLastError()) != hipSuccess) return e;
@@ -1535,7 +1787,7 @@
   hipLaunchKernelGGL(k_msm_items, dim3((n_items + 15) / 16), dim3(kQuadBlock), 0, stream, runs, n_items, mw, kt, bcomb);
   if ((e = hipGetLastError()) != hipSuccess) return e;
   hipLaunchKernelGGL((k_msm_horner<SR, true>), dim3((p.groups + 15) / 16), dim3(64), 0, stream, nullptr, n, mw, p,
-                     runs.group_run0, runs.n_runs);
+                     runs.group_run0, runs.n_runs, (const uint8_t *)nullptr, 0u);
   if ((e = hipGetLastError()) != hipSuccess) return e;
   return launch_comb_fallback<SR>(sig, key_slot, runs.order, n, w, kt, bcomb, out, aligned, mw.group_ok, p.m_log2,
                                   stream);
diff --git a/tendermint_amd/csrc/split.h b/tendermint_amd/csrc/split.h
--- /dev/null
+++ b/tendermint_amd/csrc/split.h
@@ -0,0 +1,25 @@
+#pragma once
+#include <stdint.h>
+#include "curve25519.h"
+
+namespace tmv {
+
+TMV_HD uint32_t split_windows(uint32_t W) { return (W + 1) / 2; }
+
+struct SplitSlot {
+  uint32_t window;
+  uint32_t hi;
+};
+TMV_HD SplitSlot split_slot(uint32_t w, uint32_t Ws, bool split) {
+  SplitSlot s;
+  s.hi = split && w >= Ws ? 1u : 0u;
+  s.window = s.hi ? w - Ws : w;
+  return s;
+}
+
+TMV_HD uint32_t split_max_for(uint32_t m, uint32_t want) {
+  const uint32_t most = (m - 1) / 2;
+  return want < most ? want : most;
+}
+
+}
diff --git a/tendermint_amd/csrc/tmverify_runtime.cpp b/tendermint_amd/csrc/tmverify_runtime.cpp
--- a/tendermint_amd/csrc/tmverify_runtime.cpp
+++ b/tendermint_amd/csrc/tmverify_runtime.cpp
@@ -412,6 +412,12 @@
   const char *e = tmv::ab_knob("TMV_RS_WEIGHT");
   return e ? atof(e) : kRunningSumWeight;
 }
+static std::atomic<uint32_t> g_split_groups{tmv::kMsmSplitGroups};
+static std::atomic<uint32_t> g_split_max{tmv::kMsmSplitMax};
+static uint32_t split_max() {
+  const char *e = tmv::ab_knob("TMV_SPLIT_MAX");
+  return e ? (uint32_t)strtoul(e, nullptr, 10) : g_split_max.load(std::memory_order_relaxed);
+}
 tmv::MsmParams msm_params(uint32_t n, uint32_t m_log2, uint32_t c, bool merged = false, bool ed_only = false,
                           int sub = -1) {
   const uint32_t lmin = tmv::locate_min_entries();
@@ -431,6 +437,14 @@
   if (g_msm_chunk == 16 || g_msm_chunk == 32) p.L = g_msm_chunk;
   if (g_msm_parts && g_msm_parts <= p.H && !(g_msm_parts & (g_msm_parts - 1))) p.P = g_msm_parts;
   p.sub = merged ? 0 : (sub < 0 ? (tmv::subcheck_enabled(m_log2) ? 1 : 0) : (uint32_t)sub);
+  const uint32_t sg = g_split_groups.load(std::memory_order_relaxed);
+  const uint32_t smax = tmv::split_max_for(p.m(), split_max());
+  if (!merged && ed_only && smax && (sg == 1 || (p.P == 1 && p.groups >= sg)) &&
+      2ull * n + 2 + (uint64_t)p.groups * smax < (1ull << 31)) {
+    p.split = 1;
+    p.split_max = smax;
+    p.P = 1;
+  }
   return p;
 }
 
@@ -649,7 +663,24 @@
     e = hipMemcpy(d.d_secp_gtab, gt.data(), gt.size() * sizeof(uint32_t), hipMemcpyHostToDevice);
     if (e != hipSuccess) { set_error("hipMemcpy(secp gtab)", e); return TMV_ERR_NO_DEVICE; }
   }
-  std::vector<tmv::fe> bq(2 * 4 * tmv::kBaseQuadEntries);
+  std::vector<tmv::fe> bq(2 * 4 * tmv::kBaseQuadEntries + 4 * 6);
+  for (uint32_t c = 4; c <= 9; c++) {
+    tmv::ge_p3 B;
+    tmv::ed25519_base_point(B);
+    const uint32_t sh = c * tmv::split_windows((254 + c - 1) / c);
+    for (uint32_t d = 0; d < sh; d++) {
+      tmv::ge_p1p1 t;
+      tmv::ge_p3_dbl(t, B);
+      tmv::ge_p1p1_to_p3(B, t);
+    }
+    tmv::ge_precomp pc;
+    tmv::ge_p3_to_precomp(pc, B);
+    tmv::fe *o = &bq[4 * (2 * tmv::kBaseQuadEntries + (c - 4))];
+    o[0] = pc.ymx;
+    o[1] = pc.ypx;
+    o[2] = pc.xy2d;
+    tmv::fe_one(o[3]);
+  }
   {
     tmv::ge_p3 B;
     tmv::ed25519_base_point(B);
@@ -743,9 +774,9 @@
   if (!d.ent_tried) {
     d.ent_tried = true;
     void *p = nullptr;
-    if (hipMalloc(&p, 32) != hipSuccess) {
+    if (hipMalloc(&p, 64) != hipSuccess) {
       (void)hipGetLastError();
-    } else if (hipMemset(p, 0, 32) != hipSuccess) {
+    } else if (hipMemset(p, 0, 64) != hipSuccess) {
       (void)hipGetLastError();
       (void)hipFree(p);
     } else {
@@ -1325,6 +1356,14 @@
   }
   if (name && !strcmp(name, "key_merge")) {
     tmv::set_key_merge(value != 0);
+    return 0;
+  }
+  if (name && !strcmp(name, "split_groups")) {
+    g_split_groups = value <= 0 ? tmv::kMsmSplitGroups : (uint32_t)value;
+    return 0;
+  }
+  if (name && !strcmp(name, "split_max")) {
+    g_split_max = value <= 0 ? tmv::kMsmSplitMax : (uint32_t)value;
     return 0;
   }
   set_error("unknown internal option");
@@ -2138,6 +2177,24 @@
   return 0;
 }
 
+int tmv_split_stats(tmv_ctx *ctx, uint64_t *groups_split, uint64_t *high_points) {
+  if (!ctx) return TMV_ERR_ARG;
+  uint64_t t[2] = {0, 0};
+  for (auto &d : ctx->devs) {
+    std::lock_guard<std::mutex> lk(d->mu);
+    if (!d->ent_total) continue;
+    unsigned long long v[6] = {0, 0, 0, 0, 0, 0};
+    hipError_t e = hipSetDevice(d->id);
+    if (e == hipSuccess) e = hipMemcpy(v, d->ent_total, sizeof(v), hipMemcpyDeviceToHost);
+    if (e != hipSuccess) { set_error("split counters", e); return TMV_ERR_NO_DEVICE; }
+    t[0] += v[4];
+    t[1] += v[5];
+  }
+  if (groups_split) *groups_split = t[0];
+  if (high_points) *high_points = t[1];
+  return 0;
+}
+
 int tmv_group_fail_stats(tmv_ctx *ctx, uint64_t *groups_failed, uint64_t *groups_located, uint64_t *fallback_entries) {
   if (!ctx) return TMV_ERR_ARG;
   uint64_t t[3] = {0, 0, 0};
```
